# gsc74/DipGenie

Measured on AMD Instinct MI355X. Metric: dp_state_cells_per_s, higher is better.
Workload: dtype int32

## Files before the change

dipgenie_amd/csrc/dg_dp.hpp:

```cpp
#pragma once
#include <condition_variable>
#include <atomic>
#include <map>
#include <mutex>
#include <thread>
#include <tuple>

#include "dg_internal.hpp"

namespace dgi {

constexpr int32_t NEG_INF = INT32_MIN / 4;
constexpr uint32_t BP_NONE = 0xFFFFFFFFu;
constexpr int MAX_K = 1 << 15;
constexpr int BP_MAX_RANK = 255;
constexpr int COOP_MIN = 8;
constexpr int HEAVY_INLINE = 8;
constexpr int ROWX_MAX = 64;
constexpr int DELTA_PER_BLOCK = 256 * 16;
constexpr int DELTA_PAD = 8;
constexpr int32_t CHAIN_CORRUPT = INT32_MIN;
constexpr int64_t DELTA_MAX = 65535, COLOUR_LIST_MAX = 16383;
inline bool colour_lists_fit_delta(int64_t max_hom, int64_t max_het) {
    return max_hom <= COLOUR_LIST_MAX && max_het <= COLOUR_LIST_MAX && 2 * max_hom + 4 * max_het <= DELTA_MAX;
}

struct LevelDesc {
    int32_t a0, k;
    int32_t b0, k2;
    uint32_t in_base;
    int32_t T;
    int64_t delta_off;
    int64_t bp_off;
    int32_t grp_first, ngroups;
    int32_t dead_first, ndead;
    int64_t slot_first;
    int32_t fast_ok, nblocks;
    int32_t heavy_first, n_heavy;
    int32_t bp_wide, bp_nt;
    int64_t rowx_off;
    int32_t rowx_stride;
    int16_t heavy_in[HEAVY_INLINE];
    int32_t dmax;
};

struct TraceOut { int32_t value, s_het, n_e, overflow, corrupt, path_score; };
struct ChainState { int32_t i, j, r, value; };
struct BudgetSlot { int32_t chain, budget, planes, pad_; };
constexpr int BUDGET_SYNC_STRIDE = 128;
constexpr int BUDGET_HELPER_BLOCKS = 80;
struct ColourCsr { const int64_t *hom_off, *het_off; const int32_t *hom_col, *het_col; };

struct SweepArgs {
    const LevelDesc *descs;
    const uint32_t *in_off, *in_edge, *grp_begin;
    const int32_t *in_dst, *dead_cols;
    const uint16_t *delta, *delta_zero;
    char *ring;
    size_t slot_bytes, pad_bytes;
    uint16_t *bp;
    unsigned long long *digest;
    int RP;
    int *progress;
    int flip;
};

struct FastArgs {
    const uint4 *rowrec;
    const uint2 *slots;
    const uint32_t *in_edge, *rowx;
    const int32_t *dead_cols;
    const uint16_t *delta, *delta_zero;
    char *ring;
    uint16_t *bp;
    unsigned long long *digest;
    int RP, pad_bytes;
    uint32_t buf_bytes;
    uint32_t slot_bytes;
    int *progress;
    int flip;
#ifdef DG_SWEEP_PROBE
    unsigned long long *probe;
#endif
};

inline std::atomic<int> &dp_states_on_device(int device) { static std::atomic<int> n[64]; return n[device & 63]; }

struct SweepVariant {
    int rc;
    bool general, coop;
    int index() const;
    std::string name() const;
    bool exists() const;
    static int count();
    static SweepVariant at(int index);
};
constexpr int PAIR_MAX_INDEG = 8;
constexpr int PAIR_MAX_WIDTH = 255;
constexpr int PAIR_MAX_T = 2047;
constexpr int PAIR_RCS[] = {1, 2, 4};
constexpr int N_PAIR_RCS = (int)(sizeof PAIR_RCS / sizeof PAIR_RCS[0]);
constexpr int PAIR_BIG_MAX_INDEG = 32;
constexpr int PAIR_BIG_INLINE = 8;
constexpr uint32_t PAIR_ROW_BIG = 15;
struct PairDesc {
    int32_t l, nblocks;
    int32_t k0, k1, k2;
    int32_t dmax;
    int64_t row_first;
    int64_t slot_first;
    int32_t n_big, dmax_light;
    int64_t big_first;
    uint8_t big_in[PAIR_BIG_INLINE];
};
struct PairHist {
    int64_t n[2 * N_PAIR_RCS] = {};
    void add(const PairHist &o, int64_t sign = 1) { for (int q = 0; q < 2 * N_PAIR_RCS; ++q) n[q] += sign * o.n[q]; }
};

struct SweepHist {
    std::vector<int64_t> n = std::vector<int64_t>((size_t)SweepVariant::count(), 0);
    void add(const SweepHist &o, int64_t sign = 1) { for (size_t q = 0; q < n.size(); ++q) n[q] += sign * o.n[q]; }
};

struct DpOptions {
    int64_t side_stream = -1;
    int64_t plane_limit = 1;
    int64_t want_digest = 0;
    int64_t use_fast = 1;
    int64_t adaptive_rc = 1;
    int64_t use_coop = 1;
    int64_t max_blocks = 1024;
    int64_t segment_cells = 0;
    int64_t host_threads = 16;
    int64_t test_poison_level = 0, test_poison_byte = 0xFF;
    int64_t test_force_rc = 0;
    int64_t host_tables = 0;
    int64_t bp_nt_min_cells = 262144;
    int64_t graph_batch = -1;
    int64_t warm_ahead = 128;
    int64_t sync_every = 0;
    int64_t l2_prefetch = 6;
    int64_t use_lean_chain = 1;
    int64_t delta_overlap = 1;
    int64_t pf_far = 128;
    int64_t use_rowx = 1;
    int64_t delta_cap_entries = (int64_t)4 << 30;
    int64_t rc_cap = 65536, rc_t0_ns = 3000, rc_tg_ps = 20000, rc_tw_ps = 50;
    int64_t chunk_units_cfg = (int64_t)4 << 30;
    int64_t score_slab_bytes = (int64_t)256 << 20;
    int64_t partner_slab_bytes = (int64_t)4 << 30;
    int64_t partner_wide = 0;
    int64_t pair_levels = 1;
    int64_t pair_min = 4096;
    int64_t pair_fanin = 1;
    int64_t pair_fanin_min = 4096;
    int64_t pair_fanin_max_big = 4, pair_fanin_max_indeg = PAIR_BIG_MAX_INDEG;
    int64_t pair_digest = 0;
    int64_t test_force_pair_rc = 0;
    int64_t joint_state_bytes = (int64_t)8 << 30;
    int64_t genotype_table_bytes = (int64_t)256 << 20;
    int64_t genotype_table_lanes = 0;
    int64_t genotype_table_tile_keys = 2048;
    int64_t genotype_table_scan_tiles = 1024;
    int64_t objective_lds_bytes = 131072;
};

struct DpState {
    explicit DpState(int dev) : device(dev) { ++dp_states_on_device(device); }
    ~DpState() { --dp_states_on_device(device); }
    const int device;
    DpOptions opt;
    bool side_stream_ok() const { return opt.side_stream < 0 ? dp_states_on_device(device).load() <= 1 : opt.side_stream != 0; }
    DpState(const DpState &) = delete;
    DpState &operator=(const DpState &) = delete;
    int32_t nV = 0, L = 0, R = 0, RP = 0, cap = 0;
    bool loaded = false;
    bool lean_chain = false;
    std::vector<hipEvent_t> delta_piece_ev;
    std::vector<int32_t> delta_piece_level;
    int delta_piece_next = 0;
    hipStream_t pf_stream = nullptr;
    hipEvent_t pf_ev = nullptr;
    int pf_seq = 0;
    bool pf_active = false;
    int pf_tested = 0;
    std::vector<int> seg_begin;
    std::vector<int64_t> ckpt_off;
    bool graph_failed = false;
    typedef std::tuple<int, int, const void *, int> GraphKey;
    struct Batch { hipGraphExec_t exec = nullptr; SweepHist hist; PairHist pair_hist; int64_t n_launch = 0; int flips = 0; };
    std::map<GraphKey, Batch> graphs;
    bool all_fast = false;
    size_t state_alloc_bytes = 0;
    std::vector<LevelDesc> descs;
    uint64_t cells = 0, relaxations = 0, edge_pairs = 0, colour_entries = 0;
    int64_t total_units = 0, max_level_units = 0;
    int64_t max_level_cells = 0, delta_entries = 0, n_delta_blocks = 0, pad_front = 0;
    std::vector<int64_t> level_units;
    std::vector<int32_t> dwin_t, level_win;
    int cur_win = -1;
    std::vector<int32_t> dtrans_host;
    std::vector<int64_t> dblk_first_host;
    int64_t delta_buf_entries = 0;
    std::vector<int32_t> level_dmax;
    int64_t n_grp = 0, n_dead = 0, n_heavy_rows = 0, n_slot_records = 0, n_rowx_words = 0, n_dtrans = 0, n_edges = 0;
    DevBuf d_descs, d_in_off, d_in_edge, d_in_dst, d_hom_off, d_het_off, d_hom_col, d_het_col, d_eflag, d_eself;
    std::vector<PairDesc> pairs;
    std::vector<int32_t> pair_at;
    DevBuf d_pairs, d_pair_at, d_prow, d_pslots, d_pbig, d_pbig_rows;
    PairHist pair_hist;
    DevBuf d_delta, d_bp, d_ring, d_digest, d_dblk_first, d_dtrans, d_grp, d_dead, d_heavy, d_rowrec, d_rowx, d_slots, d_ckpt, d_pfctl;
#ifdef DG_SWEEP_PROBE
    DevBuf d_probe;
#endif
    std::vector<uint64_t> digest_host;
    SweepHist launch_hist;
    dg_dp_timing timing;
    hipEvent_t ev[4] = {nullptr, nullptr, nullptr, nullptr};
    struct Pool {
        std::mutex mu;
        std::condition_variable cv;
        std::vector<void *> chunks;
        size_t chunk_units = (size_t)DpOptions().chunk_units_cfg;
        size_t target = 0;
        size_t cap_chunks = 0;
        bool running = false, failed = false, paused = false;
        std::thread th;
    } pool;
    std::vector<int> chunk_begin;
    int seg_chunks = 1;
    DevBuf d_sink, d_ch_path, d_ch_state, d_ch_sync, d_ch_trace, d_ch_edges, d_ch_tab;
    std::vector<int32_t> sink_host;
    std::vector<BudgetSlot> tab_host;
    int n_groups = 0;
    mutable int walk_seq = 0;
    DevBuf d_sc_paths, d_sc_out, d_sc_err;
    DevBuf d_pt_pairs, d_pt_bud, d_pt_val, d_pt_out, d_pt_err, d_pt_bp, d_pt_scores;
    DevBuf d_pt_state;
    int32_t pt_route = 0;
    int64_t pt_route_cells = 0;
    DevBuf d_mg_levels, d_mg_vertex;
    bool run_ok = false;
    DevBuf d_ans_paths, d_ans_cnt;
    DevBuf d_cm_class, d_cm_out;
    bool ob_dict = false;
    int64_t ob_ch = 0, ob_ct = 0;
    DevBuf d_ob_hom_rank, d_ob_het_rank, d_ob_paths, d_ob_out, d_ob_err, d_ob_bits;
    int64_t jt_stats[8] = {0, 0, 0, 0, 0, 0, 0, 0};
    int64_t ph_stats[6] = {0, 0, 0, 0, 0, 0};
    int64_t phb_stats[10] = {0, 0, 0, 0, 0, 0, 0, 0, 0, 0};
    int64_t rb_stats[7] = {0, 0, 0, 0, 0, 0, 0};
    int64_t rbb_stats[9] = {0, 0, 0, 0, 0, 0, 0, 0, 0};
    DevBuf d_pins;
    bool run_pinned = false;
    int64_t pin_stats[5] = {0, 0, 0, 0, 0};
};

inline ColourCsr colour_csr(const DpState &S) {
    return ColourCsr{S.d_hom_off.as<int64_t>(), S.d_het_off.as<int64_t>(), S.d_hom_col.as<int32_t>(), S.d_het_col.as<int32_t>()};
}

void pool_request(DpState &S, int device, size_t target);
void pool_trim(DpState &S, size_t keep);
inline void pool_clear(DpState &S) { pool_trim(S, 0); }
void *pool_wait(DpState &S, size_t c);
struct PoolPause {
    DpState &S;
    explicit PoolPause(DpState &s);
    ~PoolPause();
};
void graphs_clear(DpState &S);
double wall_s();

int dp_load(dg_ctx *c, const dg_dp_graph *g);
int dp_build_tables_device(dg_ctx *c, const dg_dp_graph *g, DpState &S, std::vector<int32_t> &dtrans, std::vector<int64_t> &dblk_first, int &max_k);
int dp_table_digest(dg_ctx *c, uint64_t *out, int n);
int dp_build_pairs(dg_ctx *c, const dg_dp_graph *g, DpState &S);

void delta_launch_edge_flags(const DpState &S, hipStream_t s);
const uint16_t *delta_launch_window(DpState &S, int w, hipStream_t s);
const uint16_t *delta_launch_overlapped(DpState &S, hipStream_t s);
void delta_overlap_free(DpState &S);

struct SweepLaunch {
    SweepArgs A;
    FastArgs F;
    bool small_state = true;
    int rc_sel = 0;
    bool digest = false;
    int rp_active = 0;
    SweepHist hist;
    PairHist pair_hist;
    bool pairs_ok = false;
    int flip = 0;
};
void sweep_prepare(const DpState &S, SweepLaunch &X);
void sweep_init_state(const DpState &S, hipStream_t s);
int sweep_launch_level(const DpState &S, SweepLaunch &X, int l, hipStream_t s);
int sweep_launch_pair(const DpState &S, SweepLaunch &X, int l, hipStream_t s);
std::string pair_variant_name(int q);
void sweep_warm_tables(const DpState &S, const SweepLaunch &X, int q0, int q1, hipStream_t s);
int sweep_prefetch_begin(DpState &S, const SweepLaunch &X, int lb, int le, bool delta_resident, hipStream_t s);
void sweep_prefetch_end(DpState &S, int le, hipStream_t s);
void sweep_prefetch_free(DpState &S);

void trace_launch_warm_rows(const DpState &S, int lb, int le, hipStream_t s);
void trace_launch_chains(const DpState &S, int n, int l_hi, int l_lo, const uint16_t *bp_biased, const int32_t *final_val, hipStream_t s);
void trace_launch_finish_chain(const DpState &S, const uint2 *path, int32_t *edges, const ChainState *st, TraceOut *out, hipStream_t s);
void trace_debug_report(const DpState &S, int n);

void budgets_launch_sink_copy(const DpState &S, const int32_t *sink_state, hipStream_t s);
int budgets_reserve(DpState &S, int n);
int budgets_prepare(DpState &S, const int32_t *budgets, int n, hipStream_t s);
void budgets_launch_finish(const DpState &S, int n, hipStream_t s);
int budgets_find_chain(const char *fn, const DpState *S, int32_t budget, int &chain);
void budgets_launch_expand(const DpState &S, int chain, int swap, int32_t *out, int32_t *cnt, hipStream_t s);
int dp_get_answer_paths(dg_ctx *c, int32_t budget, int32_t *paths);

int dp_score_paths(dg_ctx *c, const int32_t *paths, int64_t n_pairs, dg_dp_pair_score *out);
int score_pair_blocks(const DpState &S);
void score_launch_pairs(const DpState &S, const int32_t *pairs, int64_t n, int32_t *out, unsigned long long *err, hipStream_t s);

int dp_objective_paths(dg_ctx *c, const int32_t *paths, int64_t n_pairs, dg_dp_pair_objective *out);
int dp_answer_objectives(dg_ctx *c, const int32_t *budgets, int32_t n_budgets, dg_dp_pair_objective *out);
int64_t objective_lds_limit(const dg_ctx *c);

int dp_best_partners(dg_ctx *c, const int32_t *given, int64_t n, const int32_t *budgets, int32_t *partners, dg_dp_partner *out);

int dp_partner_marginals(dg_ctx *c, const int32_t *given, int64_t n, const int32_t *budgets, dg_dp_level_margin *levels, int32_t *vertex_values);
int dp_call_margins(dg_ctx *c, int32_t budget, const int32_t *vertex_class, dg_dp_call_margin *levels, int32_t *paths);

struct PinSet {
    std::vector<int32_t> off;
    const dg_dp_pin *d_pins = nullptr;
    int64_t n_mask = 0, n_pairs_split = 0, n_batches_plain = 0;
    bool has(int l) const { return off[(size_t)l + 1] > off[(size_t)l]; }
    bool any_in(int l0, int l1) const { return off[(size_t)l1] > off[(size_t)l0]; }
};
int pins_prepare(const char *fn, const DpState &S, const dg_dp_pin *pins, int64_t n, PinSet &P, DevBuf &buf);
void pins_launch_mask(const DpState &S, PinSet &P, int level, int32_t *state, hipStream_t s);
void pins_launch_joint_mask(PinSet &P, int level, int32_t *state, int k, int planes, hipStream_t s);

int dp_genotype_margins(dg_ctx *c, bool pinned, const dg_dp_pin *pins, int64_t n_pins, const int32_t *called, int64_t n, int32_t budget, const int32_t *vertex_class,
                        dg_dp_genotype_margin *levels, int32_t *vertex_values, int32_t *best_value);
int dp_genotype_table(dg_ctx *c, bool pinned, const dg_dp_pin *pins, int64_t n_pins, int32_t budget, const int32_t *vertex_class, const int32_t *called, int64_t n,
                      dg_dp_genotype_margin *levels, int64_t *level_off, dg_dp_genotype_entry **entries, int64_t *n_entries, int32_t *best_value);
int dp_genotype_margins_budgets(dg_ctx *c, const dg_dp_pin *pins, int64_t n_pins, const int32_t *called, const int32_t *budgets, int64_t n, const int32_t *vertex_class,
                                dg_dp_genotype_margin *levels, int32_t *best_values);
int dp_genotype_stats(dg_ctx *c, int64_t *out, int n);
int dp_phase_margins(dg_ctx *c, const int32_t *called, int32_t budget, const int32_t *vertex_class, dg_dp_phase_margin *records, int64_t *n_records, int32_t *best_value);
int dp_phase_stats(dg_ctx *c, int64_t *out, int n);
int dp_phase_margins_budgets(dg_ctx *c, const int32_t *called, const int32_t *budgets, int64_t n, const int32_t *vertex_class, dg_dp_phase_margin *records, int64_t *record_off,
                             int32_t *best_values);
int dp_phase_budget_stats(dg_ctx *c, int64_t *out, int n);
int dp_recombination_margins(dg_ctx *c, int32_t budget, const int32_t *called, int64_t n, dg_dp_recombination_margin *records, int32_t *called_out, int32_t *best_value);
int dp_recombination_stats(dg_ctx *c, int64_t *out, int n);
int dp_recombination_margins_budgets(dg_ctx *c, const int32_t *budgets, int64_t n, const int32_t *called, dg_dp_recombination_margin *records, int32_t *called_out,
                                     int32_t *best_values);
int dp_recombination_budget_stats(dg_ctx *c, int64_t *out, int n);

}
```

dipgenie_amd/csrc/dg_dp_pairs.hip:

```cpp
#include <sched.h>

#include <algorithm>
#include <cstdlib>
#include <memory>

#include "dg_dp.hpp"

namespace dgi {

static int cpu_share() {
    int64_t n = (int64_t)std::max(1u, std::thread::hardware_concurrency());
    cpu_set_t set;
    if (sched_getaffinity(0, sizeof set, &set) == 0) n = std::min<int64_t>(n, std::max(1, CPU_COUNT(&set)));
    if (FILE *f = fopen("/sys/fs/cgroup/cpu.max", "r")) {
        long long quota = 0, period = 0;
        if (fscanf(f, "%lld %lld", &quota, &period) == 2 && quota > 0 && period > 0) n = std::min<int64_t>(n, (quota + period - 1) / period);
        fclose(f);
    }
    return (int)std::max<int64_t>(n, 1);
}

template <class F>
static void parallel_blocks(int64_t n, int64_t block, int nt, F f) {
    std::atomic<int64_t> next{0};
    auto work = [&]() {
        for (;;) {
            const int64_t b = next.fetch_add(block);
            if (b >= n) return;
            f(b, std::min(n, b + block));
        }
    };
    std::vector<std::thread> th;
    for (int t = 1; t < nt && (int64_t)t * block < n; ++t) th.emplace_back(work);
    work();
    for (std::thread &t : th) t.join();
}

int dp_build_pairs(dg_ctx *c, const dg_dp_graph *g, DpState &S) {
    S.pairs.clear(); S.pair_at.clear();
    S.d_pairs.release(); S.d_pair_at.release(); S.d_prow.release(); S.d_pslots.release(); S.d_pbig.release(); S.d_pbig_rows.release();
    const int L = S.L, nV = S.nV;
    if (!S.opt.pair_levels || (int64_t)(L - 1) / 2 < std::max<int64_t>(S.opt.pair_min, 1) || (int)S.dwin_t.size() != 2 || S.RP > 0x1FFF) return DG_OK;
    const double t0 = wall_s();
    std::vector<uint32_t> in_off((size_t)nV + 1, 0), in_edge((size_t)g->out_off[nV]);
    DG_HIP(hipMemcpyAsync(in_off.data(), S.d_in_off.p, 4 * in_off.size(), hipMemcpyDeviceToHost, c->stream));
    if (!in_edge.empty()) DG_HIP(hipMemcpyAsync(in_edge.data(), S.d_in_edge.p, 4 * in_edge.size(), hipMemcpyDeviceToHost, c->stream));
    DG_HIP(hipStreamSynchronize(c->stream));
    const int nt = (int)std::max<int64_t>(1, std::min<int64_t>({(int64_t)16, S.opt.host_threads, (int64_t)cpu_share()}));
    auto indeg = [&](int v) { return (int)(in_off[v + 1] - in_off[v]); };
    auto level_ok = [&](int l) {
        const LevelDesc &d = S.descs[l];
        return d.fast_ok == 1 && d.ndead == 0 && d.k2 <= PAIR_MAX_WIDTH && d.T <= PAIR_MAX_T && !d.bp_wide;
    };
    struct LevelSum { int32_t cmin, cmax, cmax_light, n_big; };
    std::vector<uint16_t> comp((size_t)nV, 0);
    std::vector<LevelSum> sum((size_t)L, LevelSum{0, 0, 0, 0});
    parallel_blocks(std::max(L - 2, 0), 512, nt, [&](int64_t q0, int64_t q1) {
        for (int l = (int)q0 + 2; l < (int)q1 + 2; ++l) {
            if (!level_ok(l - 1) || !level_ok(l)) continue;
            const LevelDesc &d = S.descs[l];
            LevelSum s{1 << 30, 0, 0, 0};
            for (int v = d.b0; v < d.b0 + d.k2; ++v) {
                int n = 0;
                for (uint32_t e = in_off[v]; e < in_off[v + 1]; ++e) n += indeg(d.a0 + (int)(in_edge[e] & 0x7FFFu));
                comp[(size_t)v] = (uint16_t)n;
                s.cmin = std::min(s.cmin, n); s.cmax = std::max(s.cmax, n);
                if (n > PAIR_MAX_INDEG) ++s.n_big; else s.cmax_light = std::max(s.cmax_light, n);
            }
            sum[(size_t)l] = s;
        }
    });
    const int max_big = (int)std::min<int64_t>(S.opt.pair_fanin_max_big, PAIR_MAX_WIDTH), max_indeg = (int)std::min<int64_t>(S.opt.pair_fanin_max_indeg, PAIR_BIG_MAX_INDEG);
    auto choose = [&](bool fanin, std::vector<PairDesc> &pairs, std::vector<int32_t> &at) {
        int64_t n_fanin = 0;
        pairs.clear(); at.assign((size_t)L, -1);
        for (int l = 2; l < L; ++l) {
            const LevelSum &s = sum[(size_t)l];
            if (s.cmin < 1) continue;
            if (s.cmax > PAIR_MAX_INDEG && !(fanin && s.cmax <= max_indeg && s.n_big <= max_big)) continue;
            const LevelDesc &d = S.descs[l];
            PairDesc p{};
            p.l = l; p.k0 = S.descs[l - 1].k; p.k1 = d.k; p.k2 = d.k2; p.dmax = s.cmax; p.n_big = s.n_big; p.dmax_light = s.cmax_light;
            n_fanin += s.n_big > 0;
            at[(size_t)l] = (int32_t)pairs.size(); at[(size_t)l - 1] = -2;
            pairs.push_back(p);
            ++l;
        }
        return n_fanin;
    };
    std::vector<int32_t> at;
    std::vector<PairDesc> pairs;
    int64_t n_fanin = choose(false, pairs, at);
    if (S.opt.pair_fanin) {
        std::vector<int32_t> at_f;
        std::vector<PairDesc> pairs_f;
        const int64_t nf = choose(true, pairs_f, at_f);
        if (nf >= std::max<int64_t>(S.opt.pair_fanin_min, 1)) { pairs.swap(pairs_f); at.swap(at_f); n_fanin = nf; }
    }
    if ((int64_t)pairs.size() < std::max<int64_t>(S.opt.pair_min, 1)) return DG_OK;
    const int64_t NP = (int64_t)pairs.size();
    parallel_blocks(NP, 256, nt, [&](int64_t q0, int64_t q1) {
        for (int64_t q = q0; q < q1; ++q) {
            PairDesc &p = pairs[(size_t)q];
            const LevelDesc &d2 = S.descs[p.l];
            uint32_t used = 0;
            int32_t nb = 1;
            for (int v = d2.b0; v < d2.b0 + d2.k2; ++v) {
                const uint32_t n = comp[(size_t)v];
                if (used + n > 64) { ++nb; used = 0; }
                used += n;
            }
            p.nblocks = nb;
        }
    });
    int64_t n_rows = 0, n_blocks = 0, n_big = 0;
    for (PairDesc &p : pairs) {
        p.row_first = n_rows * PAIR_MAX_INDEG; p.slot_first = n_blocks * 64; p.big_first = n_big;
        n_rows += p.k2; n_blocks += p.nblocks; n_big += p.n_big;
    }
    const size_t prow_words = 2 * (size_t)PAIR_MAX_INDEG * (size_t)n_rows, pslot_words = 4 * 64 * (size_t)n_blocks, pbig_words = 2 * (size_t)PAIR_BIG_MAX_INDEG * (size_t)n_big;
    std::unique_ptr<uint32_t[]> prow(new uint32_t[prow_words + 1]), pslots(new uint32_t[pslot_words + 1]), pbig(new uint32_t[pbig_words + 1]);
    std::unique_ptr<int32_t[]> big_rows(new int32_t[(size_t)n_big + 1]);
    parallel_blocks(NP, 64, nt, [&](int64_t q0, int64_t q1) {
        for (int64_t q = q0; q < q1; ++q) {
            PairDesc &p = pairs[(size_t)q];
            const LevelDesc &d2 = S.descs[p.l], &d1 = S.descs[p.l - 1];
            uint32_t *const pr = prow.get() + 2 * p.row_first, *const pb = pbig.get() + 2 * (size_t)PAIR_BIG_MAX_INDEG * (size_t)p.big_first;
            uint32_t *blk = pslots.get() + 4 * p.slot_first;
            int32_t *const br = big_rows.get() + p.big_first;
            uint32_t used = 0, maxdv = 1, h = 0;
            auto close_block = [&]() {
                uint32_t steps = 0;
                while ((1u << steps) < maxdv) ++steps;
                for (uint32_t s = used; s < 64; ++s) { blk[4 * s] = 0xFFFFFFFFu; blk[4 * s + 1] = 0; blk[4 * s + 2] = 0; blk[4 * s + 3] = 0; }
                for (uint32_t s = 0; s < 64; ++s) blk[4 * s + 2] |= steps << 16;
                blk += 4 * 64; used = 0; maxdv = 1;
            };
            for (int c2 = 0; c2 < d2.k2; ++c2) {
                const int v = d2.b0 + c2;
                const uint32_t n = comp[(size_t)v];
                const bool big = n > (uint32_t)PAIR_MAX_INDEG;
                if (used + n > 64) close_block();
                uint32_t *const light = pr + 2 * (size_t)PAIR_MAX_INDEG * (size_t)c2;
                uint32_t *const rec = big ? pb + 2 * (size_t)PAIR_BIG_MAX_INDEG * h : light;
                const uint32_t cap = big ? PAIR_BIG_MAX_INDEG : PAIR_MAX_INDEG, ru1_shift = big ? 27 : 25;
                uint32_t t = 0;
                for (uint32_t e2 = in_off[v]; e2 < in_off[v + 1]; ++e2) {
                    const uint32_t m = in_edge[e2] & 0x7FFFu, w2 = in_edge[e2] >> 31, r2 = e2 - in_off[v];
                    const int mv = d2.a0 + (int)m;
                    for (uint32_t e1 = in_off[mv]; e1 < in_off[mv + 1]; ++e1, ++t) {
                        const uint32_t src = in_edge[e1] & 0x7FFFu, w1 = in_edge[e1] >> 31, r1 = e1 - in_off[mv];
                        const uint32_t i2 = e2 - d2.in_base, i1 = e1 - d1.in_base;
                        rec[2 * t] = src | (w1 << 15) | (m << 16) | (w2 << 24) | (n << 25);
                        rec[2 * t + 1] = i2 | (i1 << 11) | (r2 << 22) | (r1 << ru1_shift);
                        uint32_t *const sl = blk + 4 * (used + t);
                        sl[0] = src | (w1 << 15) | (m << 16) | (w2 << 24);
                        sl[1] = i2 | (i1 << 16);
                        sl[2] = r2 | (r1 << 8) | ((uint32_t)c2 << 20);
                        sl[3] = 0;
                    }
                }
                for (; t < cap; ++t) { rec[2 * t] = n << 25; rec[2 * t + 1] = 0; }
                if (big) {
                    for (t = 0; t < (uint32_t)PAIR_MAX_INDEG; ++t) { light[2 * t] = PAIR_ROW_BIG << 25; light[2 * t + 1] = 0; }
                    br[h] = c2;
                    if (h < (uint32_t)PAIR_BIG_INLINE) p.big_in[h] = (uint8_t)c2;
                    ++h;
                }
                used += n; maxdv = std::max(maxdv, n);
            }
            close_block();
        }
    });
    auto up = [&](DevBuf &b, const void *src, size_t bytes) -> int {
        if (int rc = b.ensure(bytes + 16)) return rc;
        if (bytes) DG_HIP(hipMemcpyAsync(b.p, src, bytes, hipMemcpyHostToDevice, c->stream));
        return DG_OK;
    };
    if (int rc = up(S.d_pairs, pairs.data(), sizeof(PairDesc) * pairs.size())) return rc;
    if (int rc = up(S.d_pair_at, at.data(), 4 * at.size())) return rc;
    if (int rc = up(S.d_prow, prow.get(), 4 * prow_words)) return rc;
    if (int rc = up(S.d_pslots, pslots.get(), 4 * pslot_words)) return rc;
    if (int rc = up(S.d_pbig, pbig.get(), 4 * pbig_words)) return rc;
    if (int rc = up(S.d_pbig_rows, big_rows.get(), 4 * (size_t)n_big)) return rc;
    DG_HIP(hipStreamSynchronize(c->stream));
    if (getenv("DG_DEBUG"))
        fprintf(stderr, "[dipgenie_hip] load: %zu level pairs (%.1f %% of the launches), %lld of them with big rows (%lld big rows), composed tables %.1f MB, built in %.3f s by %d threads\n",
                pairs.size(), 100.0 * (double)pairs.size() / std::max(1, L - 1), (long long)n_fanin, (long long)n_big, 4e-6 * (double)(prow_words + pslot_words + pbig_words), wall_s() - t0, nt);
    S.pairs.swap(pairs); S.pair_at.swap(at);
    return DG_OK;
}

}
```

dipgenie_amd/csrc/dg_dp_run.hip:

```cpp
#include <algorithm>
#include <cstdlib>
#include <cstring>
#include <ctime>

#include "dg_dp.hpp"

namespace dgi {

constexpr int DELTA_NO_PIECES = 1 << 30;

double wall_s() { struct timespec ts; clock_gettime(CLOCK_MONOTONIC, &ts); return ts.tv_sec + 1e-9 * ts.tv_nsec; }

void graphs_clear(DpState &S) {
    for (auto &kv : S.graphs) if (kv.second.exec) (void)hipGraphExecDestroy(kv.second.exec);
    S.graphs.clear();
}

void dp_state_free(DpState *s) {
    if (!s) return;
    graphs_clear(*s);
    sweep_prefetch_free(*s);
    delta_overlap_free(*s);
    { std::unique_lock<std::mutex> lk(s->pool.mu); s->pool.target = 0; }
    s->pool.cv.notify_all();
    if (s->pool.th.joinable()) s->pool.th.join();
    const double tf0 = wall_s();
    for (void *q : s->pool.chunks) (void)hipFree(q);
    if (getenv("DG_DEBUG")) fprintf(stderr, "[dipgenie_hip] destroy: %zu lattice chunks freed in %.3f s\n", s->pool.chunks.size(), wall_s() - tf0);
    for (auto &e : s->ev) if (e) (void)hipEventDestroy(e);
    delete s;
}

void pool_request(DpState &S, int device, size_t target) {
    std::unique_lock<std::mutex> lk(S.pool.mu);
    S.pool.target = std::max(target, S.pool.chunks.size());
    if (S.pool.running || S.pool.chunks.size() >= S.pool.target) return;
    if (S.pool.th.joinable()) { lk.unlock(); S.pool.th.join(); lk.lock(); }
    S.pool.running = true;
    S.pool.failed = false;
    DpState *Sp = &S;
    S.pool.th = std::thread([Sp, device]() {
        (void)hipSetDevice(device);
        for (;;) {
            size_t bytes;
            {
                std::unique_lock<std::mutex> lk2(Sp->pool.mu);
                Sp->pool.cv.wait(lk2, [&] { return !Sp->pool.paused || Sp->pool.chunks.size() >= Sp->pool.target; });
                if (Sp->pool.chunks.size() >= Sp->pool.target) { Sp->pool.running = false; Sp->pool.cv.notify_all(); return; }
                bytes = Sp->pool.chunk_units * 2;
            }
            void *q = nullptr;
            const hipError_t e = hipMalloc(&q, bytes);
            std::unique_lock<std::mutex> lk2(Sp->pool.mu);
            if (e != hipSuccess) { (void)hipGetLastError(); Sp->pool.failed = true; Sp->pool.running = false; Sp->pool.cv.notify_all(); return; }
            Sp->pool.chunks.push_back(q);
            Sp->pool.cv.notify_all();
            lk2.unlock();
            std::this_thread::sleep_for(std::chrono::milliseconds(1));
        }
    });
}
PoolPause::PoolPause(DpState &s) : S(s) { std::unique_lock<std::mutex> lk(S.pool.mu); S.pool.paused = true; }
PoolPause::~PoolPause() { { std::unique_lock<std::mutex> lk(S.pool.mu); S.pool.paused = false; } S.pool.cv.notify_all(); }
void pool_trim(DpState &S, size_t keep) {
    { std::unique_lock<std::mutex> lk(S.pool.mu); S.pool.target = std::min(std::min(S.pool.target, keep), S.pool.chunks.size()); }
    S.pool.cv.notify_all();
    if (S.pool.th.joinable()) S.pool.th.join();
    std::unique_lock<std::mutex> lk(S.pool.mu);
    while (S.pool.chunks.size() > keep) { (void)hipFree(S.pool.chunks.back()); S.pool.chunks.pop_back(); }
    S.pool.running = false;
}
void *pool_wait(DpState &S, size_t c) {
    std::unique_lock<std::mutex> lk(S.pool.mu);
    S.pool.cv.wait(lk, [&] { return S.pool.chunks.size() > c || S.pool.failed || !S.pool.running; });
    return S.pool.chunks.size() > c ? S.pool.chunks[c] : nullptr;
}

namespace {

struct Run {
    dg_ctx *c;
    DpState &S;
    hipStream_t s;
    SweepLaunch X;
    int64_t n_launch = 0;
    int next_warm = 0;
    double host_enqueue_s = 0;
    int n_chains = 1;
    std::vector<uint16_t *> pool_base;
    PinSet *P;

    Run(dg_ctx *c_, DpState &S_, PinSet *P_ = nullptr) : c(c_), S(S_), s(c_->stream), P(P_) { sweep_prepare(S, X); }
    int n_win() const { return (int)S.dwin_t.size() - 1; }
    int32_t *state_ptr(int level) const { return (int32_t *)(S.d_ring.as<char>() + (size_t)((level & 1) ^ X.flip) * S.state_alloc_bytes) + S.pad_front; }
    size_t level_cells(int level) const {
        const int64_t k = level == 0 ? 1 : S.descs[level].k2;
        return (size_t)(k * k * S.RP);
    }
    void load_window(int w) { X.A.delta = X.F.delta = delta_launch_window(S, w, s); }

    int issue_levels(int l0, int l1, int lb, int le) {
        for (int l = l0; l < l1; ++l) {
            if (S.level_win[l] >= 0 && S.level_win[l] != S.cur_win) load_window(S.level_win[l]);
            if (S.opt.warm_ahead > 0 && l >= next_warm && (l == lb || !(S.pf_active && S.opt.pf_far > 0))) {
                const int q0 = l == lb ? l : (int)std::min<int64_t>(l + S.opt.warm_ahead, le), q1 = (int)std::min<int64_t>(l + 2 * S.opt.warm_ahead, le);
                if (q1 > q0) sweep_warm_tables(S, X, q0, q1, s);
            }
            if (l >= next_warm) next_warm = l + (int)std::max<int64_t>(S.opt.warm_ahead, 1);
            const bool pair_here = X.pairs_ok && l + 1 < l1 && S.pair_at[l + 1] >= 0;
            if (pair_here && !(P && P->has(l))) {
                if (S.level_win[l + 1] >= 0 && S.level_win[l + 1] != S.cur_win) load_window(S.level_win[l + 1]);
                if (int rc = sweep_launch_pair(S, X, ++l, s)) return rc;
            } else {
                if (pair_here) ++P->n_pairs_split;
                if (int rc = sweep_launch_level(S, X, l, s)) return rc;
            }
            ++n_launch;
            if (P && P->has(l)) pins_launch_mask(S, *P, l, state_ptr(l), s);
            if (S.opt.sync_every > 0 && n_launch % S.opt.sync_every == 0) DG_HIP(hipStreamSynchronize(s));
        }
        return DG_OK;
    }

    int sweep_range(int lb, int le, uint16_t *bp_biased) {
        X.A.bp = bp_biased; X.F.bp = bp_biased;
        next_warm = lb;
        if (int rc = sweep_prefetch_begin(S, X, lb, le, n_win() == 1, s)) return rc;
        const int64_t gb = S.opt.graph_batch >= 0 ? S.opt.graph_batch : 1000;
        for (int l0 = lb; l0 < le;) {
            const int pf_key = ((S.pf_active && S.opt.pf_far > 0) ? 1 : 0) | (X.flip << 1) | (X.rp_active << 2);
            const bool graph_ok = gb > 0 && n_win() == 1 && S.opt.sync_every == 0 && !S.graph_failed;
            const int l1 = graph_ok ? (int)std::min<int64_t>((int64_t)l0 + gb, le) : le;
            const bool pinned_batch = P && P->any_in(l0, l1);
            if (graph_ok && pinned_batch) ++P->n_batches_plain;
            const bool use_graph = graph_ok && !pinned_batch;
            while (S.delta_piece_next < (int)S.delta_piece_level.size() && S.delta_piece_level[S.delta_piece_next] < l1) {
                DG_HIP(hipStreamWaitEvent(s, S.delta_piece_ev[S.delta_piece_next], 0));
                ++S.delta_piece_next;
            }
            const DpState::GraphKey key(l0, l1, (const void *)bp_biased, pf_key);
            DpState::Batch *slot = nullptr;
            bool capturing = false;
            if (use_graph) {
                slot = &S.graphs[key];
                if (slot->exec) {
                    DG_HIP(hipGraphLaunch(slot->exec, s));
                    X.hist.add(slot->hist); X.pair_hist.add(slot->pair_hist);
                    n_launch += slot->n_launch; X.flip ^= slot->flips; l0 = l1;
                    continue;
                }
                if (hipStreamBeginCapture(s, hipStreamCaptureModeThreadLocal) == hipSuccess) capturing = true;
                else { (void)hipGetLastError(); S.graph_failed = true; continue; }
            }
            const int64_t n_launch_before = n_launch;
            const SweepHist hist_before = X.hist;
            const PairHist pair_hist_before = X.pair_hist;
            const int flip_before = X.flip;
            if (int rc = issue_levels(l0, l1, lb, le)) {
                if (capturing) {
                    hipGraph_t cg = nullptr;
                    (void)hipStreamEndCapture(s, &cg);
                    if (cg) (void)hipGraphDestroy(cg);
                    (void)hipGetLastError();
                    S.graphs.erase(key);
                }
                return rc;
            }
            if (capturing) {
                hipGraph_t cg = nullptr;
                const bool ok = hipStreamEndCapture(s, &cg) == hipSuccess && cg && hipGraphInstantiate(&slot->exec, cg, nullptr, nullptr, 0) == hipSuccess;
                if (cg) (void)hipGraphDestroy(cg);
                if (!ok) {
                    (void)hipGetLastError();
                    slot->exec = nullptr; S.graph_failed = true; n_launch = n_launch_before; X.hist = hist_before; X.pair_hist = pair_hist_before; X.flip = flip_before;
                    continue;
                }
                slot->hist = X.hist;
                slot->hist.add(hist_before, -1);
                slot->pair_hist = X.pair_hist;
                slot->pair_hist.add(pair_hist_before, -1);
                slot->n_launch = n_launch - n_launch_before; slot->flips = X.flip ^ flip_before;
                DG_HIP(hipGraphLaunch(slot->exec, s));
            }
            l0 = l1;
        }
        sweep_prefetch_end(S, le, s);
        return DG_OK;
    }

    int wait_for_chunks() {
        if (S.d_bp.p) return DG_OK;
        const double tw0 = wall_s();
        const size_t need = (size_t)std::min(S.seg_chunks, (int)S.chunk_begin.size() - 1);
        if (!pool_wait(S, need - 1)) { set_error("back-pointer lattice: hipMalloc of a %.1f GB chunk failed", S.pool.chunk_units * 2 / 1e9); return DG_ERR_OOM; }
        std::unique_lock<std::mutex> lk(S.pool.mu);
        for (size_t q = 0; q < need; ++q) pool_base.push_back((uint16_t *)S.pool.chunks[q]);
        if (getenv("DG_DEBUG")) fprintf(stderr, "[dipgenie_hip] run: waited %.3f s for lattice chunks\n", wall_s() - tw0);
        return DG_OK;
    }

    std::tuple<int, int, uint16_t *> chunk(int ch, int c0) const {
        const int lb = S.d_bp.p ? 1 : S.chunk_begin[ch], le = S.d_bp.p ? S.L : S.chunk_begin[ch + 1];
        return {lb, le, (S.d_bp.p ? S.d_bp.as<uint16_t>() : pool_base[ch - c0]) - S.descs[lb].bp_off};
    }

    int sweep_and_walk(int c0, int c1, bool from_sink, bool mark_forward_end) {
        for (int ch = c0; ch < c1; ++ch) {
            const auto [lb, le, bp] = chunk(ch, c0);
            const double th0 = wall_s();
            if (int rc = sweep_range(lb, le, bp)) return rc;
            host_enqueue_s += wall_s() - th0;
        }
        if (mark_forward_end) { DG_HIP(hipEventRecord(S.ev[2], s)); budgets_launch_sink_copy(S, state_ptr(S.L - 1), s); }
        if (S.opt.test_poison_level > 0 && S.opt.test_poison_level < S.L)
            for (int ch = c0; ch < c1; ++ch) {
                const auto [lb, le, bp] = chunk(ch, c0);
                const int lp = (int)S.opt.test_poison_level;
                if (lp >= lb && lp < le) DG_HIP(hipMemsetAsync(bp + S.descs[lp].bp_off, (int)S.opt.test_poison_byte, 2 * (size_t)S.level_units[lp], s));
            }
        for (int ch = c1 - 1; ch >= c0; --ch) {
            const auto [lb, le, bp] = chunk(ch, c0);
            trace_launch_warm_rows(S, lb, le, s);
            const int32_t *final_val = from_sink && ch == c1 - 1 ? state_ptr(S.L - 1) : (const int32_t *)nullptr;
            trace_launch_chains(S, n_chains, le - 1, lb, bp, final_val, s);
        }
        return DG_OK;
    }

    int forward_and_trace() {
        const int n_seg = (int)S.seg_begin.size() - 1, n_chunks_all = (int)S.chunk_begin.size() - 1;
        DG_HIP(hipEventRecord(S.ev[0], s));
        S.cur_win = -1;
        S.delta_piece_next = DELTA_NO_PIECES;
        if (n_win() == 1 && S.n_delta_blocks > 0) X.A.delta = X.F.delta = delta_launch_overlapped(S, s);
        DG_HIP(hipEventRecord(S.ev[1], s));
        if (S.opt.want_digest) DG_HIP(hipMemsetAsync(S.d_digest.p, 0, 8 * (size_t)S.L, s));
#ifdef DG_SWEEP_PROBE
        {
            std::vector<unsigned long long> init((size_t)S.L * 8, 0ULL);
            for (int l = 0; l < S.L; ++l) init[(size_t)l * 8] = ~0ULL;
            DG_HIP(hipMemcpy(S.d_probe.p, init.data(), 8 * init.size(), hipMemcpyHostToDevice));
        }
#endif
        sweep_init_state(S, s);
        X.pairs_ok = !S.pairs.empty() && S.opt.pair_levels && n_seg == 1 && n_win() == 1 && (!X.digest || S.opt.pair_digest) && S.opt.use_fast && S.opt.adaptive_rc && S.opt.test_force_rc == 0 &&
                     X.small_state && X.rp_active == S.RP;
        if (n_seg == 1) {
            if (int rc = sweep_and_walk(0, S.d_bp.p ? 1 : n_chunks_all, true, true)) return rc;
        } else {
            int64_t planes_swept = 0;
            for (int sg = 0; sg < n_seg; ++sg) {
                if (sg > 0)
                    DG_HIP(hipMemcpyAsync(S.d_ckpt.as<int32_t>() + S.ckpt_off[sg], state_ptr(S.seg_begin[sg] - 1),
                                          4 * level_cells(S.seg_begin[sg] - 1), hipMemcpyDeviceToDevice, s));
                if (int rc = sweep_range(S.seg_begin[sg], S.seg_begin[sg + 1], nullptr)) return rc;
            }
            DG_HIP(hipEventRecord(S.ev[2], s));
            budgets_launch_sink_copy(S, state_ptr(S.L - 1), s);
            X.digest = false;
            for (int sg = n_seg - 1; sg >= 0; --sg) {
                const int lb = S.seg_begin[sg];
                if (sg > 0)
                    DG_HIP(hipMemcpyAsync(state_ptr(lb - 1), S.d_ckpt.as<int32_t>() + S.ckpt_off[sg], 4 * level_cells(lb - 1), hipMemcpyDeviceToDevice, s));
                else
                    sweep_init_state(S, s);
                const int c0 = sg * S.seg_chunks, c1 = std::min(n_chunks_all, c0 + S.seg_chunks);
                if (int rc = sweep_and_walk(c0, c1, sg == n_seg - 1, false)) return rc;
                if (S.opt.plane_limit && sg > 0) {
                    std::vector<ChainState> cs((size_t)n_chains);
                    DG_HIP(hipMemcpyAsync(cs.data(), S.d_ch_state.p, sizeof(ChainState) * cs.size(), hipMemcpyDeviceToHost, s));
                    DG_HIP(hipStreamSynchronize(s));
                    int planes = 1;
                    for (const ChainState &q : cs) {
                        if (q.value == NEG_INF) continue;
                        planes = std::max(planes, (q.value != CHAIN_CORRUPT && q.r >= 0 && q.r < S.RP) ? q.r + 1 : S.RP);
                    }
                    X.rp_active = planes;
                    planes_swept += (int64_t)planes * (S.seg_begin[sg] - S.seg_begin[sg - 1]);
                }
            }
            if (getenv("DG_DEBUG") && S.opt.plane_limit) fprintf(stderr, "[dipgenie_hip] run: second pass swept %.1f %% of the (level, plane) pairs before the last segment\n",
                                                              100.0 * (double)planes_swept / std::max(1.0, (double)S.RP * (S.seg_begin[n_seg - 1] - 1)));
        }
        budgets_launch_finish(S, n_chains, s);
        DG_HIP(hipEventRecord(S.ev[3], s));
        DG_HIP(hipGetLastError());
        return DG_OK;
    }
};

}

static int emit_result(const DpState &S, const TraceOut &to, const int32_t *edges, dg_dp_result *res, int budget) {
    char who[32] = "";
    if (budget >= 0) snprintf(who, sizeof who, " (budget %d)", budget);
    if (to.value == CHAIN_CORRUPT || to.corrupt) { set_error("back-pointer lattice is corrupt: the chain walk left its level (a level was not swept?)%s", who); return DG_ERR_STATE; }
    if (to.value != NEG_INF && to.path_score != to.value) {
        set_error("traceback path scores %d but the DP value is %d: sweep, lattice and walk disagree%s", to.path_score, to.value, who); return DG_ERR_STATE;
    }
    if (to.overflow || to.n_e > S.cap) { set_error("traceback edge list overflow (%d > %d)%s", to.n_e, S.cap, who); return DG_ERR_STATE; }
    res->value = to.value; res->s_het = to.s_het;
    res->cells = S.cells; res->relaxations = S.relaxations;
    std::vector<int> order(to.n_e);
    for (int q = 0; q < to.n_e; ++q) order[q] = q;
    std::stable_sort(order.begin(), order.end(), [&](int a, int b) { return edges[a] < edges[b]; });
    int n1 = 0, n2 = 0;
    for (int q : order) {
        const int from = edges[S.cap + q], tov = edges[2 * S.cap + q];
        if (edges[3 * S.cap + q] == 0) { if (n1 < res->cap && res->p1_from && res->p1_to) { res->p1_from[n1] = from; res->p1_to[n1] = tov; } ++n1; }
        else { if (n2 < res->cap && res->p2_from && res->p2_to) { res->p2_from[n2] = from; res->p2_to[n2] = tov; } ++n2; }
    }
    res->n_p1 = n1; res->n_p2 = n2;
    return DG_OK;
}

static int dp_run(dg_ctx *c, const int32_t *budgets, int n_budgets, dg_dp_result *res, bool name_budget, PinSet *P = nullptr) {
    DpState &S = *c->dp;
    Run run(c, S, P);
    hipStream_t s = c->stream;
    if (int rc = run.wait_for_chunks()) return rc;
    std::vector<TraceOut> to((size_t)n_budgets);
    std::vector<int32_t> edges(4 * (size_t)S.cap * (size_t)n_budgets);
    S.run_ok = false;
    S.run_pinned = P != nullptr;
    if (int rc = budgets_prepare(S, budgets, n_budgets, s)) return rc;
    run.n_chains = n_budgets;
    S.sink_host.clear();
    const int rc_run = run.forward_and_trace();
    S.launch_hist = run.X.hist;
    S.pair_hist = run.X.pair_hist;
    if (rc_run) return rc_run;
    DG_HIP(hipMemcpyAsync(to.data(), S.d_ch_trace.p, sizeof(TraceOut) * to.size(), hipMemcpyDeviceToHost, s));
    DG_HIP(hipMemcpyAsync(edges.data(), S.d_ch_edges.p, 4 * edges.size(), hipMemcpyDeviceToHost, s));
    std::vector<int32_t> sink((size_t)S.RP);
    DG_HIP(hipMemcpyAsync(sink.data(), S.d_sink.p, 4 * sink.size(), hipMemcpyDeviceToHost, s));
    if (S.opt.want_digest) {
        S.digest_host.assign(S.L, 0);
        DG_HIP(hipMemcpyAsync(S.digest_host.data(), S.d_digest.p, 8 * (size_t)S.L, hipMemcpyDeviceToHost, s));
    }
    DG_HIP(hipStreamSynchronize(s));
    S.sink_host.swap(sink);
#ifdef DG_SWEEP_PROBE
    if (const char *po = getenv("DG_PROBE_OUT")) {
        std::vector<unsigned long long> pr((size_t)S.L * 8);
        DG_HIP(hipMemcpy(pr.data(), S.d_probe.p, 8 * pr.size(), hipMemcpyDeviceToHost));
        if (FILE *f = fopen(po, "wb")) { fwrite(pr.data(), 8, pr.size(), f); fclose(f); }
    }
#endif
    if (getenv("DG_DEBUG") && S.lean_chain) trace_debug_report(S, n_budgets);
    if (getenv("DG_DEBUG") && S.pf_stream) {
        int w[4] = {0, 0, 0, 0};
        if (hipStreamSynchronize(S.pf_stream) == hipSuccess && hipMemcpy(w, S.d_pfctl.p, sizeof w, hipMemcpyDeviceToHost) == hipSuccess)
            fprintf(stderr, "[dipgenie_hip] run: L2 table prefetcher covered %d levels (since load)\n", w[2]);
    }
    if (getenv("DG_DEBUG"))
        fprintf(stderr, "[dipgenie_hip] run: host issued %lld sweep launches in %.1f ms (%.2f us each)\n", (long long)run.n_launch, 1e3 * run.host_enqueue_s,
                1e6 * run.host_enqueue_s / (double)std::max<int64_t>(run.n_launch, 1));
    DG_HIP(hipEventElapsedTime(&S.timing.delta_ms, S.ev[0], S.ev[1]));
    DG_HIP(hipEventElapsedTime(&S.timing.forward_ms, S.ev[1], S.ev[2]));
    DG_HIP(hipEventElapsedTime(&S.timing.traceback_ms, S.ev[2], S.ev[3]));
    DG_HIP(hipEventElapsedTime(&S.timing.total_ms, S.ev[0], S.ev[3]));
    S.timing.n_forward_launches = run.n_launch;
    S.timing.n_segments = (int32_t)S.seg_begin.size() - 1;
    S.timing.n_chunks = (int32_t)S.chunk_begin.size() - 1;
    for (int q = 0; q < n_budgets; ++q)
        if (int rc = emit_result(S, to[q], edges.data() + 4 * (size_t)S.cap * (size_t)q, res + q, name_budget ? budgets[q] : -1)) return rc;
    S.run_ok = true;
    return DG_OK;
}

static int check_budgets(const char *fn, const DpState *Sp, const int32_t *budgets, int32_t n, const dg_dp_result *results) {
    if (!Sp || !Sp->loaded) { set_error("%s: no graph loaded", fn); return DG_ERR_STATE; }
    if (!budgets || !results || n <= 0) { set_error("%s: budgets, results and n_budgets > 0 are required", fn); return DG_ERR_ARG; }
    std::vector<char> seen((size_t)Sp->RP, 0);
    for (int q = 0; q < n; ++q) {
        const int b = budgets[q];
        if (b < 0 || b > Sp->R) { set_error("%s: budget %d (entry %d) outside 0..%d, the R of the loaded graph", fn, b, q, Sp->R); return DG_ERR_ARG; }
        if (seen[b]) { set_error("%s: budget %d listed twice", fn, b); return DG_ERR_ARG; }
        seen[b] = 1;
        if (results[q].cap < b + 2) { set_error("%s: results[%d].cap = %d, budget %d needs %d", fn, q, results[q].cap, b, b + 2); return DG_ERR_ARG; }
    }
    return DG_OK;
}

static int dp_run_budgets(dg_ctx *c, const int32_t *budgets, int32_t n, dg_dp_result *results) {
    if (int rc = check_budgets("dg_dp_run_budgets", c->dp, budgets, n, results)) return rc;
    return dp_run(c, budgets, n, results, true);
}

static int dp_run_pinned(dg_ctx *c, const dg_dp_pin *pins, int64_t n_pins, const int32_t *budgets, int32_t n, dg_dp_result *results) {
    if (n_pins == 0) return dp_run_budgets(c, budgets, n, results);
    if (int rc = check_budgets("dg_dp_run_pinned", c->dp, budgets, n, results)) return rc;
    DpState &S = *c->dp;
    if (S.opt.want_digest) {
        set_error("dg_dp_run_pinned: option digest is 1: the sweep accumulates a level's digest before the level's mask runs, so the digest would describe another DP");
        return DG_ERR_STATE;
    }
    PinSet P;
    if (int rc = pins_prepare("dg_dp_run_pinned", S, pins, n_pins, P, S.d_pins)) return rc;
    const int rc = dp_run(c, budgets, n, results, true, &P);
    int64_t n_levels = 0;
    for (int l = 1; l < S.L; ++l) n_levels += P.has(l);
    const int64_t st[5] = {n_pins, n_levels, P.n_mask, P.n_pairs_split, P.n_batches_plain};
    memcpy(S.pin_stats, st, sizeof st);
    return rc;
}

static int dp_run_single(dg_ctx *c, dg_dp_result *res) {
    if (!c->dp || !c->dp->loaded) { set_error("dg_dp_run: no graph loaded"); return DG_ERR_STATE; }
    if (!res) { set_error("dg_dp_run: null result"); return DG_ERR_ARG; }
    const int32_t budget = c->dp->R;
    return dp_run(c, &budget, 1, res, false);
}

}

extern "C" int dg_dp_load_graph(dg_ctx *c, const dg_dp_graph *g) {
    if (int rc = dgi::bind(c)) return rc;
    return dgi::dp_load(c, g);
}
extern "C" int dg_dp_run(dg_ctx *c, dg_dp_result *r) {
    if (int rc = dgi::bind(c)) return rc;
    return dgi::dp_run_single(c, r);
}
extern "C" int dg_dp_run_budgets(dg_ctx *c, const int32_t *budgets, int32_t n_budgets, dg_dp_result *results) {
    if (int rc = dgi::bind(c)) return rc;
    return dgi::dp_run_budgets(c, budgets, n_budgets, results);
}
extern "C" int dg_dp_run_pinned(dg_ctx *c, const dg_dp_pin *pins, int64_t n_pins, const int32_t *budgets, int32_t n_budgets, dg_dp_result *results) {
    if (int rc = dgi::bind(c)) return rc;
    return dgi::dp_run_pinned(c, pins, n_pins, budgets, n_budgets, results);
}
extern "C" int dg_dp_get_pin_stats(dg_ctx *c, int64_t *out, int n) {
    if (!c || !c->dp) { dgi::set_error("dg_dp_get_pin_stats: no state"); return DG_ERR_STATE; }
    if (!out || n < 5) { dgi::set_error("dg_dp_get_pin_stats: out with n >= 5 entries is required"); return DG_ERR_ARG; }
    memcpy(out, c->dp->pin_stats, sizeof c->dp->pin_stats);
    return DG_OK;
}
extern "C" int dg_dp_get_budget_values(dg_ctx *c, int32_t *out, int32_t n) {
    if (!c || !c->dp || !out) { dgi::set_error("dg_dp_get_budget_values: no state"); return DG_ERR_STATE; }
    const std::vector<int32_t> &v = c->dp->sink_host;
    if (v.empty()) { dgi::set_error("dg_dp_get_budget_values: no completed dg_dp_run / dg_dp_run_budgets on the loaded graph"); return DG_ERR_STATE; }
    if (n < (int32_t)v.size()) { dgi::set_error("dg_dp_get_budget_values: out has %d entries, R + 1 = %zu needed", n, v.size()); return DG_ERR_ARG; }
    memcpy(out, v.data(), 4 * v.size());
    return DG_OK;
}
extern "C" int dg_dp_solve_diploid(dg_ctx *c, const dg_dp_graph *g, dg_dp_result *r) {
    if (int rc = dg_dp_load_graph(c, g)) return rc;
    return dg_dp_run(c, r);
}
extern "C" int dg_dp_prealloc(dg_ctx *c, int64_t bytes) {
    if (int rc = dgi::bind(c)) return rc;
    if (!c->dp) c->dp = new dgi::DpState(c->device);
    dgi::DpState &S = *c->dp;
    if (S.pool.chunk_units != (size_t)S.opt.chunk_units_cfg) { dgi::pool_clear(S); S.pool.chunk_units = (size_t)S.opt.chunk_units_cfg; }
    const size_t chunk_bytes = S.pool.chunk_units * 2;
    if (S.pool.cap_chunks == 0) {
        size_t free_b = 0, total_b = 0;
        DG_HIP(hipMemGetInfo(&free_b, &total_b));
        S.pool.cap_chunks = std::max<size_t>(1, (size_t)(0.6 * (double)free_b) / chunk_bytes);
    }
    const size_t want_chunks = bytes > 0 ? std::min(((size_t)bytes + chunk_bytes - 1) / chunk_bytes, S.pool.cap_chunks) : S.pool.cap_chunks;
    dgi::pool_request(S, c->device, want_chunks);
    return DG_OK;
}
extern "C" int dg_dp_get_timing(dg_ctx *c, dg_dp_timing *t) {
    if (!c || !c->dp || !t) { dgi::set_error("dg_dp_get_timing: no state"); return DG_ERR_STATE; }
    *t = c->dp->timing;
    return DG_OK;
}
extern "C" int dg_dp_get_level_digest(dg_ctx *c, uint64_t *out, int64_t n) {
    if (!c || !c->dp || !out) { dgi::set_error("dg_dp_get_level_digest: no state"); return DG_ERR_STATE; }
    if ((int64_t)c->dp->digest_host.size() != n) { dgi::set_error("digest not collected (set option digest=1) or size mismatch"); return DG_ERR_STATE; }
    memcpy(out, c->dp->digest_host.data(), 8 * (size_t)n);
    return DG_OK;
}
extern "C" int dg_dp_get_table_digest(dg_ctx *c, uint64_t *out, int n) {
    if (int rc = dgi::bind(c)) return rc;
    return dgi::dp_table_digest(c, out, n);
}
extern "C" int dg_dp_get_launch_profile(dg_ctx *c, char *buf, int cap) {
    if (!c || !c->dp || !buf || cap < 2) { dgi::set_error("dg_dp_get_launch_profile: no state"); return DG_ERR_STATE; }
    std::string out;
    for (int q = 0; q < dgi::SweepVariant::count(); ++q)
        if (const int64_t n = c->dp->launch_hist.n[(size_t)q]) out += (out.empty() ? "" : " ") + dgi::SweepVariant::at(q).name() + ':' + std::to_string(n);
    if ((int)out.size() + 1 > cap) { dgi::set_error("dg_dp_get_launch_profile: buffer too small (%zu needed)", out.size() + 1); return DG_ERR_ARG; }
    memcpy(buf, out.c_str(), out.size() + 1);
    return DG_OK;
}
extern "C" int dg_dp_get_pair_profile(dg_ctx *c, char *buf, int cap) {
    if (!c || !c->dp || !buf || cap < 2) { dgi::set_error("dg_dp_get_pair_profile: no state"); return DG_ERR_STATE; }
    std::string out;
    for (int q = 0; q < 2 * dgi::N_PAIR_RCS; ++q)
        if (const int64_t n = c->dp->pair_hist.n[q]) out += (out.empty() ? "" : " ") + dgi::pair_variant_name(q) + ':' + std::to_string(n);
    if ((int)out.size() + 1 > cap) { dgi::set_error("dg_dp_get_pair_profile: buffer too small (%zu needed)", out.size() + 1); return DG_ERR_ARG; }
    memcpy(buf, out.c_str(), out.size() + 1);
    return DG_OK;
}
extern "C" int dg_dp_list_pair_variants(char *buf, int cap) {
    std::string out;
    for (int q = 0; q < dgi::N_PAIR_RCS; ++q) out += (out.empty() ? "" : " ") + dgi::pair_variant_name(q);
    if (!buf || (int)out.size() + 1 > cap) { dgi::set_error("dg_dp_list_pair_variants: buffer too small (%zu needed)", out.size() + 1); return DG_ERR_ARG; }
    memcpy(buf, out.c_str(), out.size() + 1);
    return DG_OK;
}
extern "C" int dg_dp_list_sweep_variants(char *buf, int cap) {
    std::string out;
    for (int q = 0; q < dgi::SweepVariant::count(); ++q)
        if (dgi::SweepVariant::at(q).exists()) out += (out.empty() ? "" : " ") + dgi::SweepVariant::at(q).name();
    if (!buf || (int)out.size() + 1 > cap) { dgi::set_error("dg_dp_list_sweep_variants: buffer too small (%zu needed)", out.size() + 1); return DG_ERR_ARG; }
    memcpy(buf, out.c_str(), out.size() + 1);
    return DG_OK;
}
typedef dgi::DpOptions DpO;
static const struct DpOptionKey { const char *key; int64_t DpO::*field; int64_t lo; bool nonpos_is_default; } dp_option_keys[] = {
    {"digest", &DpO::want_digest, 0, false}, {"fast", &DpO::use_fast, 0, false}, {"adaptive_rc", &DpO::adaptive_rc, 0, false}, {"coop", &DpO::use_coop, 0, false},
    {"sync_every", &DpO::sync_every, 0, false}, {"rc_t0_ns", &DpO::rc_t0_ns, 0, false}, {"rc_tg_ps", &DpO::rc_tg_ps, 0, false}, {"rc_tw_ps", &DpO::rc_tw_ps, 0, false},
    {"rc_cap", &DpO::rc_cap, 0, true}, {"max_blocks", &DpO::max_blocks, 0, true}, {"bp_nt_min_cells", &DpO::bp_nt_min_cells, 0, false}, {"warm_ahead", &DpO::warm_ahead, 0, false},
    {"graph_batch", &DpO::graph_batch, -1, false}, {"l2_prefetch", &DpO::l2_prefetch, 0, false}, {"delta_overlap", &DpO::delta_overlap, 0, false}, {"pf_far", &DpO::pf_far, 0, false},
    {"side_stream", &DpO::side_stream, -1, false}, {"plane_limit", &DpO::plane_limit, 0, false}, {"test_poison_level", &DpO::test_poison_level, 0, false},
    {"test_poison_byte", &DpO::test_poison_byte, 0, false}, {"test_force_rc", &DpO::test_force_rc, 0, false}, {"pair_digest", &DpO::pair_digest, 0, false}, {"test_force_pair_rc", &DpO::test_force_pair_rc, 0, false},
    {"score_slab_bytes", &DpO::score_slab_bytes, 0, true}, {"partner_slab_bytes", &DpO::partner_slab_bytes, 0, true},
    {"partner_wide", &DpO::partner_wide, 0, false},
    {"joint_state_bytes", &DpO::joint_state_bytes, 0, true},
    {"genotype_table_bytes", &DpO::genotype_table_bytes, 0, true}, {"genotype_table_lanes", &DpO::genotype_table_lanes, 0, false},
    {"genotype_table_tile_keys", &DpO::genotype_table_tile_keys, 256, true}, {"genotype_table_scan_tiles", &DpO::genotype_table_scan_tiles, 64, true},
    {"objective_lds_bytes", &DpO::objective_lds_bytes, 0, true},
    {"rowx", &DpO::use_rowx, 0, false}, {"lean_chain", &DpO::use_lean_chain, 0, false}, {"segment_cells", &DpO::segment_cells, 0, false},
    {"host_threads", &DpO::host_threads, 1, false}, {"host_tables", &DpO::host_tables, 0, false}, {"delta_cap_entries", &DpO::delta_cap_entries, 0, true},
    {"pair_levels", &DpO::pair_levels, 0, false}, {"pair_min", &DpO::pair_min, 1, false}, {"pair_fanin", &DpO::pair_fanin, 0, false}, {"pair_fanin_min", &DpO::pair_fanin_min, 1, false},
    {"pair_fanin_max_big", &DpO::pair_fanin_max_big, 0, false}, {"pair_fanin_max_indeg", &DpO::pair_fanin_max_indeg, 0, false},
    {"lattice_chunk_cells", &DpO::chunk_units_cfg, 1, false},
};
static int dp_option(dg_ctx *c, const char *what, const char *key, const int64_t *set, int64_t *get) {
    if (!c || !key || (!set && !get)) { dgi::set_error("%s: null", what); return DG_ERR_ARG; }
    if (!c->dp) c->dp = new dgi::DpState(c->device);
    dgi::DpState &S = *c->dp;
    if (set) dgi::graphs_clear(S);
    for (const DpOptionKey &o : dp_option_keys) {
        if (strcmp(key, o.key)) continue;
        if (!set) { *get = S.opt.*o.field; return DG_OK; }
        int64_t v = *set;
        if (o.field == &DpO::chunk_units_cfg) {
            if (v < o.lo) { dgi::set_error("lattice_chunk_cells must be positive"); return DG_ERR_ARG; }
            dgi::pool_clear(S);
            v = (int64_t)(S.pool.chunk_units = ((size_t)v + 1) & ~(size_t)1);
        }
        if (o.field == &DpO::objective_lds_bytes) v = std::min(v, dgi::objective_lds_limit(c));
        if (o.field == &DpO::partner_wide) v = std::min<int64_t>(v, 2);
        if (o.field == &DpO::genotype_table_tile_keys && v > 0) v = std::min<int64_t>(std::max<int64_t>(v / 256, 1) * 256, 2048);
        if (o.field == &DpO::genotype_table_scan_tiles && v > 0) v = std::min<int64_t>(std::max<int64_t>(v / 64, 1) * 64, 1024);
        S.opt.*o.field = o.nonpos_is_default && v <= 0 ? DpO().*o.field : v < o.lo ? o.lo : v;
        return DG_OK;
    }
    dgi::set_error("unknown option %s", key);
    return DG_ERR_ARG;
}
extern "C" int dg_dp_set_option(dg_ctx *c, const char *key, int64_t v) { return dp_option(c, "dg_dp_set_option", key, &v, nullptr); }
extern "C" int dg_dp_get_option(dg_ctx *c, const char *key, int64_t *value) { return dp_option(c, "dg_dp_get_option", key, nullptr, value); }
```

dipgenie_amd/csrc/dg_dp_sweep.hip:

```cpp
#include <algorithm>
#include <cmath>
#include <type_traits>

#include "dg_dp.hpp"

namespace dgi {

#define DG_SLOT(LEVEL) ((LEVEL) & 1)

constexpr unsigned long long DIGEST_PRED_MUL = 0x9E3779B97F4A7C15ULL;

__device__ __forceinline__ void store_bp_nt(uint16_t *p, uint32_t v) { asm volatile("global_store_short %0, %1, off nt" ::"v"(p), "v"(v) : "memory"); }
__device__ __forceinline__ uint32_t ord_rank(int eu, int ev) { return ((uint32_t)(BP_MAX_RANK - eu) << 8) | (uint32_t)(BP_MAX_RANK - ev); }

__device__ __forceinline__ unsigned long long digest_term(int value, unsigned long long o, uint32_t pred_i, uint32_t pred_j) {
    return (unsigned long long)(uint32_t)(value + 1) * (o + 1) +
           DIGEST_PRED_MUL * ((((unsigned long long)pred_i << 15) | pred_j) + 1ULL) * (o + 1);
}

__device__ __forceinline__ int lane_down1(int x) { return __builtin_amdgcn_update_dpp(x, x, 0x130 , 0xF, 0xF, false); }
__device__ __forceinline__ int lane_up1(int x) { return __builtin_amdgcn_update_dpp(x, x, 0x138 , 0xF, 0xF, false); }

struct LevelHead {
    const uint4 *rowrec_l;
    const uint2 *slots_l;
    const uint32_t *rowx_l;
    const int32_t *cur;
    const uint16_t *dm;
    int rowx_stride, RP, k, pad_bytes, dT;
    uint32_t buf_bytes;
};

__device__ __forceinline__ __amdgpu_buffer_rsrc_t state_rsrc(const int32_t *padded_base, uint32_t bytes) {
    return __builtin_amdgcn_make_buffer_rsrc((void *)padded_base, 0, bytes, 0x00020000);
}

__device__ __forceinline__ void publish_level(int *progress, int lvl) {
    if ((blockIdx.x | blockIdx.y | blockIdx.z) == 0 && threadIdx.x == 0) __hip_atomic_store(progress, lvl, __ATOMIC_RELAXED, __HIP_MEMORY_SCOPE_AGENT);
}

__device__ __forceinline__ uint32_t ord_word(int i, int j, int wu, int wv) {
    return ((uint32_t)(0x7FFF - i) << 17) | ((uint32_t)(0x7FFF - j) << 2) | ((uint32_t)wu << 1) | (uint32_t)wv;
}
__device__ __forceinline__ uint32_t bp_from_ord(uint32_t o) {
    const uint32_t i = 0x7FFFu - (o >> 17), j = 0x7FFFu - ((o >> 2) & 0x7FFFu);
    return i | (j << 15) | (((o >> 1) & 1u) << 30) | ((o & 1u) << 31);
}
template <int RC, bool DIGEST>
__device__ __forceinline__ void sweep_level_pairs(const SweepArgs &A, int lvl, int wave_id, int n_waves) {
    const LevelDesc d = A.descs[lvl];
    const int RP = A.RP;
    const int32_t *__restrict__ cur = (const int32_t *)(A.ring + (size_t)(DG_SLOT(lvl - 1) ^ A.flip) * A.slot_bytes + A.pad_bytes);
    int32_t *__restrict__ nxt = (int32_t *)(A.ring + (size_t)(DG_SLOT(lvl) ^ A.flip) * A.slot_bytes + A.pad_bytes);
    const int lane = threadIdx.x & 63;
    const int nchunk = (RP + RC - 1) / RC;
    const int64_t ntask = (int64_t)d.k2 * d.ngroups * nchunk;
    const bool has_delta = d.delta_off >= 0;
    const uint16_t *dm = has_delta ? A.delta + d.delta_off : A.delta_zero;
    const int dT = has_delta ? d.T : 0, dmask = has_delta ? -1 : 0;
    const uint32_t *gb = A.grp_begin + d.grp_first;
    unsigned long long dsum = 0;
    for (int64_t task = wave_id; task < ntask; task += n_waves) {
        const int g = (int)(task % d.ngroups);
        const int64_t rest = task / d.ngroups;
        const int rc = (int)(rest % nchunk), i2 = (int)(rest / nchunk);
        const int r0 = rc * RC;
        const uint32_t gbeg = gb[g], gend = gb[g + 1];
        const uint32_t eu0 = A.in_off[d.b0 + i2], eu1 = A.in_off[d.b0 + i2 + 1];
        int bval[RC];
        uint32_t bord[RC];
#pragma unroll
        for (int q = 0; q < RC; ++q) { bval[q] = NEG_INF; bord[q] = 0; }
        int j2 = -1 - lane;
        for (uint32_t cb = gbeg; cb < gend; cb += 64) {
            const uint32_t ev = cb + lane;
            const bool act = ev < gend;
            int j = 0, wv = 0, evr = 0;
            if (act) {
                const uint32_t pv = A.in_edge[ev];
                j = (int)(pv & 0x7FFFFFFFu); wv = (int)(pv >> 31);
                const int cv = A.in_dst[ev];
                j2 = cv - d.b0;
                if (!d.bp_wide) evr = (int)(ev - A.in_off[cv]);
            }
            const int dcol = (int)(ev - d.in_base) & dmask;
            for (uint32_t eu = eu0; eu < eu1; ++eu) {
                const uint32_t pu = A.in_edge[eu];
                const int i = (int)(pu & 0x7FFFFFFFu), wu = (int)(pu >> 31);
                if (act) {
                    const int w = wu + wv;
                    const int dl = (int)dm[(int64_t)(eu - d.in_base) * dT + dcol];
                    const uint32_t ord = d.bp_wide ? ord_word(i, j, wu, wv) : ord_rank((int)(eu - eu0), evr);
                    const int32_t *base = cur + ((int64_t)i * RP + (r0 - w)) * d.k + j;
                    int vals[RC];
#pragma unroll
                    for (int q = 0; q < RC; ++q) vals[q] = base[q * d.k];
#pragma unroll
                    for (int q = 0; q < RC; ++q) {
                        const int cand = vals[q] + dl;
                        const bool ok = (r0 + q < RP) & (r0 + q - w >= 0) & (vals[q] != NEG_INF);
                        const bool take = ok & ((cand > bval[q]) | ((cand == bval[q]) & (ord > bord[q])));
                        bval[q] = take ? cand : bval[q];
                        bord[q] = take ? ord : bord[q];
                    }
                }
            }
        }
        const int span = (int)min(gend - gbeg, 64u);
        for (int s = 1; s < span; s <<= 1) {
            const int oj2 = __shfl_down(j2, s);
            const bool same = (lane + s < 64) & (oj2 == j2);
#pragma unroll
            for (int q = 0; q < RC; ++q) {
                const int ov = __shfl_down(bval[q], s);
                const uint32_t oo = (uint32_t)__shfl_down((int)bord[q], s);
                const bool take = same & ((ov > bval[q]) | ((ov == bval[q]) & (oo > bord[q])));
                bval[q] = take ? ov : bval[q];
                bord[q] = take ? oo : bord[q];
            }
        }
        const int pj2 = __shfl_up(j2, 1);
        const bool head = (j2 >= 0) & ((lane == 0) | (pj2 != j2));
        if (head) {
#pragma unroll
            for (int q = 0; q < RC; ++q) {
                const int r2 = r0 + q;
                if (r2 < RP) {
                    const int64_t idx = ((int64_t)i2 * RP + r2) * d.k2 + j2;
                    nxt[idx] = bval[q];
                    if (A.bp) {
                        if (d.bp_wide) __builtin_nontemporal_store((uint32_t)(bval[q] == NEG_INF ? BP_NONE : bp_from_ord(bord[q])), (uint32_t *)(A.bp + d.bp_off + 2 * idx));
                        else __builtin_nontemporal_store((uint16_t)~bord[q], &A.bp[d.bp_off + idx]);
                    }
                    if (DIGEST && bval[q] != NEG_INF) {
                        const unsigned long long o = ((unsigned long long)r2 * d.k2 + i2) * d.k2 + j2;
                        uint32_t pi, pj;
                        if (d.bp_wide) { const uint32_t h = bp_from_ord(bord[q]); pi = h & 0x7FFFu; pj = (h >> 15) & 0x7FFFu; }
                        else {
                            const uint32_t ru = BP_MAX_RANK - (bord[q] >> 8), rv = BP_MAX_RANK - (bord[q] & 0xFFu);
                            pi = A.in_edge[eu0 + ru] & 0x7FFFFFFFu;
                            pj = A.in_edge[A.in_off[d.b0 + j2] + rv] & 0x7FFFFFFFu;
                        }
                        dsum += digest_term(bval[q], o, pi, pj);
                    }
                }
            }
        }
        if (g == 0 && d.ndead > 0) {
            for (int t = lane; t < d.ndead * RC; t += 64) {
                const int q = t % RC, c = A.dead_cols[d.dead_first + t / RC];
                if (r0 + q < RP) {
                    const int64_t idx = ((int64_t)i2 * RP + r0 + q) * d.k2 + c;
                    nxt[idx] = NEG_INF;
                    if (A.bp) {
                        if (d.bp_wide) __builtin_nontemporal_store((uint32_t)(BP_NONE), (uint32_t *)(A.bp + d.bp_off + 2 * idx));
                        else __builtin_nontemporal_store((uint16_t)0xFFFFu, &A.bp[d.bp_off + idx]);
                    }
                }
            }
        }
    }
    if (DIGEST && dsum) atomicAdd(&A.digest[lvl], dsum);
}

template <int RC, bool DIGEST>
__global__ __launch_bounds__(256) void dp_sweep_kernel(SweepArgs A, int lvl) {
    sweep_level_pairs<RC, DIGEST>(A, lvl, (int)(blockIdx.x * 4 + (threadIdx.x >> 6)), (int)(gridDim.x * 4));
}

__global__ void dp_init_kernel(int32_t *cur, int RP) {
    const int r = (int)(blockIdx.x * blockDim.x + threadIdx.x);
    if (r < RP) cur[r] = 0;
}


template <int RC>
__device__ __forceinline__ void relax_select(const int (&vals)[RC], int dl, uint32_t ord, int r0, int w, int RP,
                                             int (&bval)[RC], uint32_t (&bord)[RC]) {
#pragma unroll
    for (int q = 0; q < RC; ++q) {
        const int cand = vals[q] + dl;
        const bool ok = (r0 + q < RP) & (r0 + q - w >= 0) & (vals[q] != NEG_INF);
        const bool take = ok & ((cand > bval[q]) | ((cand == bval[q]) & (ord > bord[q])));
        bval[q] = take ? cand : bval[q];
        bord[q] = take ? ord : bord[q];
    }
}

__device__ __forceinline__ void merge_best(int ov, uint32_t oo, bool same, int &bv, uint32_t &bo) {
    const bool take = same & ((ov > bv) | ((ov == bv) & (oo > bo)));
    bv = take ? ov : bv;
    bo = take ? oo : bo;
}

#ifdef DG_SWEEP_PROBE
#define DG_PROBE_BEGIN unsigned long long pq[6] = {0, 0, 0, 0, 0, 0}; \
    const bool probe_on = A.probe != nullptr && blockIdx.x == 0 && blockIdx.y == 0 && (threadIdx.x >> 6) == 0 && (int)blockIdx.z < d.k2;
#define DG_PROBE(q) do { if (probe_on) { asm volatile("s_waitcnt vmcnt(0) lgkmcnt(0)" ::: "memory"); pq[q] = __builtin_amdgcn_s_memrealtime(); } } while (0)
#define DG_PROBE_END do { if (probe_on && (threadIdx.x & 63) == 0) { \
        atomicMin(&A.probe[(size_t)lvl * 8 + 0], pq[0]); atomicMax(&A.probe[(size_t)lvl * 8 + 1], pq[5]); \
        if ((int)blockIdx.z == d.k2 / 2) for (int q = 0; q < 6; ++q) A.probe[(size_t)lvl * 8 + 2 + q] = pq[q]; } } while (0)
#else
#define DG_PROBE_BEGIN
#define DG_PROBE(q) do { } while (0)
#define DG_PROBE_END do { } while (0)
#endif

template <int RC, bool DIGEST, bool GENERAL, int COOP>
__device__ __forceinline__ void sweep_task(const LevelHead &H, const FastArgs &A, const LevelDesc &d, __amdgpu_buffer_rsrc_t cur_rsrc,
                                           int32_t *__restrict__ nxt, int i2, int g, int r0, int lvl, int part = 0, uint2 *ex = nullptr) {
    const int lane = threadIdx.x & 63;
    const int RP = H.RP;
    DG_PROBE_BEGIN
    DG_PROBE(0);
    const uint4 rr = H.rowrec_l[i2];
    uint2 sl = H.slots_l[g * 64 + lane];
    const bool rowx = !GENERAL && H.rowx_stride > 0;
    uint32_t mypu = 0;
    if (rowx && lane < H.rowx_stride) mypu = H.rowx_l[i2 * H.rowx_stride + lane];
    int steps = __builtin_amdgcn_readfirstlane((int)(sl.y >> 28));
    const int j2 = (sl.x != 0xFFFFFFFFu) ? (int)((sl.x >> 16) & 0x7FFFu) : -1 - lane;
    int nblk = 1;
    if (GENERAL) {
        if (steps == 14) return;
        if (steps == 15) {
            const int col = __builtin_amdgcn_readfirstlane(j2);
            nblk = ((int)H.rowrec_l[col].y + 63) >> 6;
            steps = 6;
        }
    }
    const uint16_t *dm = H.dm;
    const int dT = H.dT;
    const bool has_delta = dT != 0;
    const int du = (int)rr.y;
    if (COOP == 1 && du > COOP_MIN) return;
    DG_PROBE(1);
    const int t_lo = COOP == 2 ? (du * part) >> 2 : 0, t_hi = COOP == 2 ? (du * (part + 1)) >> 2 : du;
    int bval[RC];
    uint32_t bord[RC];
#pragma unroll
    for (int q = 0; q < RC; ++q) { bval[q] = NEG_INF; bord[q] = 0; }
    const int64_t erow0 = (int64_t)rr.x * dT;
    const int rowbytes = H.k * 4;
    bool act = false;
    for (int blk = 0; blk < (GENERAL ? nblk : 1); ++blk) {
        if (GENERAL && blk > 0) sl = H.slots_l[(g + blk) * 64 + lane];
        const bool actb = sl.x != 0xFFFFFFFFu;
        act |= actb;
        const int j = (int)(sl.x & 0x7FFFu), wv = (int)((sl.x >> 15) & 1u);
        const int dcol = has_delta ? (int)(sl.y & 0x000FFFFFu) : 0;
        const int evr = (int)((sl.y >> 20) & 0xFFu);
        if (du <= 2) {
            if (actb && du > 0) {
                const int ia = (int)(rr.z & 0x7FFFu), wa = (int)(rr.z >> 31) + wv;
                const int ib = (int)(rr.w & 0x7FFFu), wb = (int)(rr.w >> 31) + wv;
                const int offa = ((ia * RP + (r0 - wa)) * H.k + j) * 4 + H.pad_bytes;
                const int offb = ((ib * RP + (r0 - wb)) * H.k + j) * 4 + H.pad_bytes;
                int va[RC], vb[RC];
                const int dla = (int)dm[erow0 + dcol];
                int dlb = 0;
#pragma unroll
                for (int q = 0; q < RC; ++q)
                    va[q] = __builtin_amdgcn_raw_buffer_load_b32(cur_rsrc, offa + q * rowbytes, 0, 0);
                if (du == 2) {
                    dlb = (int)dm[erow0 + dT + dcol];
#pragma unroll
                    for (int q = 0; q < RC; ++q)
                        vb[q] = __builtin_amdgcn_raw_buffer_load_b32(cur_rsrc, offb + q * rowbytes, 0, 0);
                }
                relax_select<RC>(va, dla, ord_rank(0, evr), r0, wa, RP, bval, bord);
                if (du == 2) relax_select<RC>(vb, dlb, ord_rank(1, evr), r0, wb, RP, bval, bord);
            }
        } else {
            constexpr int U = GENERAL ? (RC >= 4 ? 2 : 4) : (RC >= 8 ? 2 : (RC >= 4 ? 4 : 8));
            for (int c0 = GENERAL ? t_lo : 0; c0 < t_hi; c0 += GENERAL ? 64 : (1 << 30)) {
                const int tb = GENERAL ? c0 : t_lo, te = GENERAL ? min(c0 + 64, t_hi) : t_hi;
                if (!rowx) { mypu = 0; if (c0 + lane < te) mypu = A.in_edge[rr.x + c0 + lane]; }
                for (int t = tb; t < te; t += U) {
                    uint32_t wmask = 0;
                    if (actb) {
                        int vals[U][RC], dl[U];
#pragma unroll
                        for (int u = 0; u < U; ++u) {
                            if (t + u < te) {
                                const uint32_t p = (uint32_t)__builtin_amdgcn_readlane((int)mypu, t + u - c0);
                                wmask |= (p >> 31) << u;
                                const int iu = (int)(p & 0x7FFFFFFFu), w = (int)(p >> 31) + wv;
                                const int off = ((iu * RP + (r0 - w)) * H.k + j) * 4 + H.pad_bytes;
                                dl[u] = (int)dm[erow0 + (int64_t)(t + u) * dT + dcol];
#pragma unroll
                                for (int q = 0; q < RC; ++q)
                                    vals[u][q] = __builtin_amdgcn_raw_buffer_load_b32(cur_rsrc, off + q * rowbytes, 0, 0);
                            }
                        }
#pragma unroll
                        for (int u = 0; u < U; ++u) {
                            if (t + u < te) {
                                const int wu = (int)((wmask >> u) & 1u);
                                relax_select<RC>(vals[u], dl[u], ord_rank(t + u, evr), r0, wu + wv, RP, bval, bord);
                            }
                        }
                    }
                }
            }
        }
    }
    DG_PROBE(2);
    if (COOP == 2) {
        if (part > 0) {
#pragma unroll
            for (int q = 0; q < RC; ++q) ex[((part - 1) * RC + q) * 64 + lane] = make_uint2((uint32_t)bval[q], bord[q]);
        }
        __syncthreads();
        if (part > 0) return;
#pragma unroll
        for (int p = 0; p < 3; ++p) {
#pragma unroll
            for (int q = 0; q < RC; ++q) {
                const uint2 o = ex[(p * RC + q) * 64 + lane];
                merge_best((int)o.x, o.y, true, bval[q], bord[q]);
            }
        }
    }
    if (steps > 0) {
        const int oj2 = lane_down1(j2);
        const bool same = (lane + 1 < 64) & (oj2 == j2);
#pragma unroll
        for (int q = 0; q < RC; ++q) merge_best(lane_down1(bval[q]), (uint32_t)lane_down1((int)bord[q]), same, bval[q], bord[q]);
    }
    for (int st = 1, sh = 2; st < steps; ++st, sh <<= 1) {
        const int oj2 = __shfl_down(j2, sh);
        const bool same = (lane + sh < 64) & (oj2 == j2);
#pragma unroll
        for (int q = 0; q < RC; ++q) merge_best(__shfl_down(bval[q], sh), (uint32_t)__shfl_down((int)bord[q], sh), same, bval[q], bord[q]);
    }
    const int pj2 = lane_up1(j2);
    const bool head = act & ((lane == 0) | (pj2 != j2));
    unsigned long long dsum = 0;
    DG_PROBE(3);
    if (head) {
#pragma unroll
        for (int q = 0; q < RC; ++q) {
            const int r2 = r0 + q;
            if (r2 < RP) {
                const int idx = (i2 * RP + r2) * d.k2 + j2;
                nxt[idx] = bval[q];
                if (A.bp) { if (d.bp_nt) store_bp_nt(&A.bp[d.bp_off + idx], ~bord[q]); else A.bp[d.bp_off + idx] = (uint16_t)~bord[q]; }
                if (DIGEST && bval[q] != NEG_INF) {
                    const unsigned long long o = ((unsigned long long)r2 * d.k2 + i2) * d.k2 + j2;
                    const uint32_t ru = BP_MAX_RANK - (bord[q] >> 8), rv = BP_MAX_RANK - (bord[q] & 0xFFu);
                    const uint32_t pi = A.in_edge[rr.x + ru] & 0x7FFFFFFFu;
                    const uint32_t pj = A.in_edge[H.rowrec_l[j2].x + rv] & 0x7FFFFFFFu;
                    dsum += digest_term(bval[q], o, pi, pj);
                }
            }
        }
    }
    if (g == 0 && d.ndead > 0) {
        for (int t = lane; t < d.ndead * RC; t += 64) {
            const int q = t % RC, c = A.dead_cols[d.dead_first + t / RC];
            if (r0 + q < RP) {
                const int64_t idx = ((int64_t)i2 * RP + r0 + q) * d.k2 + c;
                nxt[idx] = NEG_INF;
                if (A.bp) { if (d.bp_nt) store_bp_nt(&A.bp[d.bp_off + idx], 0xFFFFu); else A.bp[d.bp_off + idx] = (uint16_t)0xFFFFu; }
            }
        }
    }
    if (DIGEST && dsum) atomicAdd(&A.digest[lvl], dsum);
#ifdef DG_SWEEP_PROBE
    if (probe_on) pq[4] = __builtin_amdgcn_s_memrealtime();
    DG_PROBE(5);
    DG_PROBE_END;
#endif
}

#ifndef DG_PLAIN_WG
#define DG_PLAIN_WG 256
#endif
#define DG_PLAIN_GW ((DG_PLAIN_WG / 64) < 4 ? (DG_PLAIN_WG / 64) : 4)
#define DG_PLAIN_CH ((DG_PLAIN_WG / 64) / DG_PLAIN_GW)
template <int RC, bool DIGEST, bool GENERAL>
__global__ __launch_bounds__(DG_PLAIN_WG) void dp_sweep_fast_kernel(const uint4 *rowrec_l, const uint2 *slots_l, const uint32_t *rowx_l, const int32_t *cur, const uint16_t *dm,
                                                            int rowx_stride, int nblocks, int rp_k, int pad_bytes, int dT, uint32_t buf_bytes,
                                                            FastArgs A, LevelDesc d, int lvl) {
    const LevelHead H{rowrec_l, slots_l, rowx_l, cur, dm, rowx_stride, rp_k & 0x1FFF, rp_k >> 13, pad_bytes, dT, buf_bytes};
    publish_level(A.progress, lvl);
    const int wv = (int)(threadIdx.x >> 6);
    const int g = (int)blockIdx.x * DG_PLAIN_GW + (wv % DG_PLAIN_GW);
    const int r0 = ((int)blockIdx.y * DG_PLAIN_CH + wv / DG_PLAIN_GW) * RC;
    if (g >= nblocks || r0 >= (rp_k & 0x1FFF)) return;
    int32_t *nxt = (int32_t *)(A.ring + (size_t)(DG_SLOT(lvl) ^ A.flip) * A.slot_bytes + A.pad_bytes);
    sweep_task<RC, DIGEST, GENERAL, 0>(H, A, d, state_rsrc(cur, buf_bytes), nxt, (int)blockIdx.z, g, r0, lvl);
}

template <int RC, bool DIGEST, bool GENERAL>
__global__ __launch_bounds__(256) void dp_sweep_coop_kernel(const uint4 *rowrec_l, const uint2 *slots_l, const uint32_t *rowx_l, const int32_t *cur,
                                                            int rowx_stride, int nblocks, int n_heavy, int rp_k, unsigned long long heavy_lo,
                                                            unsigned long long heavy_hi,
                                                            FastArgs A, LevelDesc d, int lvl, const uint16_t *dm, int dT, const int32_t *__restrict__ heavy_rows) {
    const LevelHead H{rowrec_l, slots_l, rowx_l, cur, dm, rowx_stride, rp_k & 0x1FFF, rp_k >> 13, A.pad_bytes, dT, A.buf_bytes};
    publish_level(A.progress, lvl);
    int32_t *nxt = (int32_t *)(A.ring + (size_t)(DG_SLOT(lvl) ^ A.flip) * A.slot_bytes + A.pad_bytes);
    const int r0 = (int)blockIdx.y * RC;
    const int zc = 4 * n_heavy;
    if ((int)blockIdx.z < zc) {
        __shared__ uint2 ex[3 * RC * 64];
        const int hz = (int)blockIdx.z;
        const int g = (int)blockIdx.x * 4 + (hz & 3);
        if (g >= nblocks) return;
        const int h = hz >> 2;
        int i2;
        if (h < 4) i2 = (int)((heavy_lo >> (16 * h)) & 0xFFFFu);
        else if (h < HEAVY_INLINE) i2 = (int)((heavy_hi >> (16 * (h - 4))) & 0xFFFFu);
        else i2 = heavy_rows[d.heavy_first + h];
        sweep_task<RC, DIGEST, GENERAL, 2>(H, A, d, state_rsrc(cur, A.buf_bytes), nxt, i2, g, r0, lvl, (int)(threadIdx.x >> 6), ex);
        return;
    }
    const int g = (int)blockIdx.x * 4 + (int)(threadIdx.x >> 6);
    if (g >= nblocks) return;
    sweep_task<RC, DIGEST, GENERAL, 1>(H, A, d, state_rsrc(cur, A.buf_bytes), nxt, (int)blockIdx.z - zc, g, r0, lvl);
}

template <int RC>
__device__ __forceinline__ void relax_pair(const int (&vals)[RC], int dl, uint32_t ord, uint32_t mid, int r0, int w, int RP,
                                           int (&bval)[RC], uint32_t (&bord)[RC], uint32_t (&bmid)[RC]) {
#pragma unroll
    for (int q = 0; q < RC; ++q) {
        const int cand = vals[q] + dl;
        const bool ok = (r0 + q < RP) & (r0 + q - w >= 0) & (vals[q] != NEG_INF);
        const bool take = ok & ((cand > bval[q]) | ((cand == bval[q]) & (ord > bord[q])));
        bval[q] = take ? cand : bval[q];
        bord[q] = take ? ord : bord[q];
        bmid[q] = take ? mid : bmid[q];
    }
}
__device__ __forceinline__ void merge_best_pair(int ov, uint32_t oo, uint32_t om, bool same, int &bv, uint32_t &bo, uint32_t &bm) {
    const bool take = same & ((ov > bv) | ((ov == bv) & (oo > bo)));
    bv = take ? ov : bv;
    bo = take ? oo : bo;
    bm = take ? om : bm;
}

struct PairHead {
    const uint4 *pslots_l;
    const int32_t *cur;
    const uint16_t *dm1, *dm2;
    int RP, k0, pad_bytes, dT1, dT2;
    uint32_t buf_bytes;
};

template <int RC, bool DIGEST, int COOP>
__device__ __forceinline__ void pair_task(const PairHead &H, const uint2 *recs, int32_t *__restrict__ nxt, uint16_t *__restrict__ bp1, uint16_t *__restrict__ bp2, int kk, int nt,
                                          int i2, int g, int r0, int lvl, unsigned long long *digest, int part = 0, uint4 *ex = nullptr) {
    const int lane = threadIdx.x & 63;
    const int RP = H.RP, k0 = H.k0, pad_bytes = H.pad_bytes, dT1 = H.dT1, dT2 = H.dT2;
    const uint16_t *dm1 = H.dm1, *dm2 = H.dm2;
    constexpr int NREC = COOP == 2 ? PAIR_BIG_MAX_INDEG : PAIR_MAX_INDEG, RU1_SHIFT = COOP == 2 ? 27 : 25, RANK_MASK = COOP == 2 ? 31 : 7;
    const uint2 rec = recs[lane & (NREC - 1)];
    const uint4 sl = H.pslots_l[g * 64 + lane];
    const __amdgpu_buffer_rsrc_t cur_rsrc = state_rsrc(H.cur, H.buf_bytes);
    const int du = __builtin_amdgcn_readfirstlane((int)(rec.x >> 25)) & (COOP == 2 ? 0x3F : 0xF);
    if (COOP == 1 && du > PAIR_MAX_INDEG) return;
    const int t_lo = COOP == 2 ? (du * part) >> 2 : 0, t_hi = COOP == 2 ? (du * (part + 1)) >> 2 : du;
    const int steps = __builtin_amdgcn_readfirstlane((int)(sl.z >> 16)) & 0xF;
    const bool act = sl.x != 0xFFFFFFFFu;
    const int j = (int)(sl.x & 0x7FFFu), wv = (int)((sl.x >> 15) & 1u) + (int)((sl.x >> 24) & 1u);
    const uint32_t lanemid = (((sl.x >> 16) & 0xFFu) << 8) | ((sl.x >> 24) & 1u);
    const int j2 = act ? (int)((sl.z >> 20) & 0xFFu) : -1 - lane;
    const int c2 = dT2 ? (int)(sl.y & 0xFFFFu) : 0, c1 = dT1 ? (int)(sl.y >> 16) : 0;
    const uint32_t ordc = ((uint32_t)(BP_MAX_RANK - (int)(sl.z & 0xFFu)) << 16) | (uint32_t)(BP_MAX_RANK - (int)((sl.z >> 8) & 0xFFu));
    int bval[RC];
    uint32_t bord[RC], bmid[RC];
#pragma unroll
    for (int q = 0; q < RC; ++q) { bval[q] = NEG_INF; bord[q] = 0; bmid[q] = 0; }
    const int rowbytes = k0 * 4;
    constexpr int U = COOP == 2 ? PAIR_MAX_INDEG : (RC >= 4 ? 4 : 8);
    for (int t = t_lo; t < t_hi; t += U) {
        if (act) {
            int vals[U][RC], dl[U];
#pragma unroll
            for (int u = 0; u < U; ++u) {
                if (t + u < t_hi) {
                    const uint32_t px = (uint32_t)__builtin_amdgcn_readlane((int)rec.x, t + u), py = (uint32_t)__builtin_amdgcn_readlane((int)rec.y, t + u);
                    const int iu = (int)(px & 0x7FFFu), w = (int)((px >> 15) & 1u) + (int)((px >> 24) & 1u) + wv;
                    const int off = ((iu * RP + (r0 - w)) * k0 + j) * 4 + pad_bytes;
                    dl[u] = (int)dm2[(int)(py & 0x7FFu) * dT2 + c2] + (int)dm1[(int)((py >> 11) & 0x7FFu) * dT1 + c1];
#pragma unroll
                    for (int q = 0; q < RC; ++q) vals[u][q] = __builtin_amdgcn_raw_buffer_load_b32(cur_rsrc, off + q * rowbytes, 0, 0);
                }
            }
#pragma unroll
            for (int u = 0; u < U; ++u) {
                if (t + u < t_hi) {
                    const uint32_t px = (uint32_t)__builtin_amdgcn_readlane((int)rec.x, t + u), py = (uint32_t)__builtin_amdgcn_readlane((int)rec.y, t + u);
                    const int w = (int)((px >> 15) & 1u) + (int)((px >> 24) & 1u) + wv;
                    const uint32_t ord = ((uint32_t)(BP_MAX_RANK - (int)((py >> 22) & RANK_MASK)) << 24) | ((uint32_t)(BP_MAX_RANK - (int)((py >> RU1_SHIFT) & RANK_MASK)) << 8) | ordc;
                    const uint32_t mid = ((((px >> 16) & 0xFFu) << 16) | ((px >> 24) & 1u)) + lanemid;
                    relax_pair<RC>(vals[u], dl[u], ord, mid, r0, w, RP, bval, bord, bmid);
                }
            }
        }
    }
    if (COOP == 2) {
        if (part > 0) {
#pragma unroll
            for (int q = 0; q < RC; ++q) ex[((part - 1) * RC + q) * 64 + lane] = make_uint4((uint32_t)bval[q], bord[q], bmid[q], 0u);
        }
        __syncthreads();
        if (part > 0) return;
#pragma unroll
        for (int p = 0; p < 3; ++p) {
#pragma unroll
            for (int q = 0; q < RC; ++q) {
                const uint4 o = ex[(p * RC + q) * 64 + lane];
                merge_best_pair((int)o.x, o.y, o.z, true, bval[q], bord[q], bmid[q]);
            }
        }
    }
    if (steps > 0) {
        const int oj2 = lane_down1(j2);
        const bool same = (lane + 1 < 64) & (oj2 == j2);
#pragma unroll
        for (int q = 0; q < RC; ++q) merge_best_pair(lane_down1(bval[q]), (uint32_t)lane_down1((int)bord[q]), (uint32_t)lane_down1((int)bmid[q]), same, bval[q], bord[q], bmid[q]);
    }
    for (int st = 1, sh = 2; st < steps; ++st, sh <<= 1) {
        const int oj2 = __shfl_down(j2, sh);
        const bool same = (lane + sh < 64) & (oj2 == j2);
#pragma unroll
        for (int q = 0; q < RC; ++q)
            merge_best_pair(__shfl_down(bval[q], sh), (uint32_t)__shfl_down((int)bord[q], sh), (uint32_t)__shfl_down((int)bmid[q], sh), same, bval[q], bord[q], bmid[q]);
    }
    const int pj2 = lane_up1(j2);
    const bool head = act & ((lane == 0) | (pj2 != j2));
    unsigned long long dsum = 0;
    if (head) {
        const int k1 = kk & 0xFF, k2 = kk >> 8;
#pragma unroll
        for (int q = 0; q < RC; ++q) {
            const int r2 = r0 + q;
            if (r2 < RP) {
                const int idx = (i2 * RP + r2) * k2 + j2;
                nxt[idx] = bval[q];
                if (bp2) {
                    const uint32_t b2 = ~(bord[q] >> 16);
                    if (nt) store_bp_nt(&bp2[idx], b2); else bp2[idx] = (uint16_t)b2;
                    if (bord[q]) {
                        const uint32_t m = bmid[q];
                        bp1[((int)(m >> 16) * RP + r2 - (int)(m & 0xFFu)) * k1 + (int)((m >> 8) & 0xFFu)] = (uint16_t)~bord[q];
                    }
                }
                if (DIGEST && bval[q] != NEG_INF) {
                    const unsigned long long o = ((unsigned long long)r2 * k2 + i2) * k2 + j2;
                    dsum += digest_term(bval[q], o, bmid[q] >> 16, (bmid[q] >> 8) & 0xFFu);
                }
            }
        }
    }
    if (DIGEST && dsum) atomicAdd(&digest[lvl], dsum);
}

template <int RC, typename... DG>
__global__ __launch_bounds__(256) void dp_sweep_pair_kernel(const uint2 *prow_l, const uint4 *pslots_l, const int32_t *cur, const uint16_t *dm1, const uint16_t *dm2,
                                                            int nblocks, int rp_k, int pad_bytes, int dT1, int dT2, uint32_t buf_bytes,
                                                            int32_t *__restrict__ nxt, uint16_t *__restrict__ bp1, uint16_t *__restrict__ bp2, int kk, int nt, int *progress, int lvl,
                                                            DG... digest) {
    constexpr bool DIGEST = sizeof...(DG) != 0;
    publish_level(progress, lvl);
    const int g = (int)blockIdx.x * 4 + (int)(threadIdx.x >> 6), r0 = (int)blockIdx.y * RC, i2 = (int)blockIdx.z;
    if (g >= nblocks) return;
    const PairHead H{pslots_l, cur, dm1, dm2, rp_k & 0x1FFF, rp_k >> 13, pad_bytes, dT1, dT2, buf_bytes};
    unsigned long long *const acc[] = {nullptr, digest...};
    pair_task<RC, DIGEST, 0>(H, prow_l + i2 * PAIR_MAX_INDEG, nxt, bp1, bp2, kk, nt, i2, g, r0, lvl, acc[sizeof...(DG)]);
}

template <int RC, typename... DG>
__global__ __launch_bounds__(256) void dp_sweep_pair_coop_kernel(const uint2 *prow_l, const uint4 *pslots_l, const uint2 *pbig_l, const int32_t *cur, const uint16_t *dm2,
                                                                 unsigned long long big_in, int nblocks, int n_big, int rp_k, int dT2,
                                                                 const uint16_t *dm1, int dT1, int pad_bytes, uint32_t buf_bytes, const int32_t *__restrict__ big_rows,
                                                                 int32_t *__restrict__ nxt, uint16_t *__restrict__ bp1, uint16_t *__restrict__ bp2, int kk, int nt, int *progress, int lvl,
                                                                 DG... digest) {
    constexpr bool DIGEST = sizeof...(DG) != 0;
    publish_level(progress, lvl);
    const PairHead H{pslots_l, cur, dm1, dm2, rp_k & 0x1FFF, rp_k >> 13, pad_bytes, dT1, dT2, buf_bytes};
    unsigned long long *const acc[] = {nullptr, digest...};
    const int r0 = (int)blockIdx.y * RC;
    const int zc = 4 * n_big;
    if ((int)blockIdx.z < zc) {
        __shared__ uint4 ex[3 * RC * 64];
        const int hz = (int)blockIdx.z;
        const int g = (int)blockIdx.x * 4 + (hz & 3);
        if (g >= nblocks) return;
        const int h = hz >> 2;
        const int i2 = h < PAIR_BIG_INLINE ? (int)((big_in >> (8 * h)) & 0xFFu) : big_rows[h];
        pair_task<RC, DIGEST, 2>(H, pbig_l + h * PAIR_BIG_MAX_INDEG, nxt, bp1, bp2, kk, nt, i2, g, r0, lvl, acc[sizeof...(DG)], (int)(threadIdx.x >> 6), ex);
        return;
    }
    const int g = (int)blockIdx.x * 4 + (int)(threadIdx.x >> 6), i2 = (int)blockIdx.z - zc;
    if (g >= nblocks) return;
    pair_task<RC, DIGEST, 1>(H, prow_l + i2 * PAIR_MAX_INDEG, nxt, bp1, bp2, kk, nt, i2, g, r0, lvl, acc[sizeof...(DG)]);
}

constexpr int WARM_RANGES = 5;
struct WarmRanges { const char *p[WARM_RANGES]; long long n16[WARM_RANGES]; };
__global__ __launch_bounds__(256) void dp_warm_tables_kernel(WarmRanges W) {
    const long long tid = (long long)blockIdx.x * blockDim.x + threadIdx.x, nth = (long long)gridDim.x * blockDim.x;
#pragma unroll
    for (int q = 0; q < WARM_RANGES; ++q) {
        const uint4 *p = (const uint4 *)W.p[q];
        for (long long i = tid; i < W.n16[q]; i += nth) { uint4 v = p[i]; asm volatile("" ::"v"(v.x), "v"(v.y), "v"(v.z), "v"(v.w)); }
    }
}

constexpr int PF_WORKGROUPS = 16, PF_FAR_WORKGROUPS = 16;
constexpr unsigned long long PF_IDLE_TICKS = 30000;
struct PfCtl { int seq, stop, levels_done, probe, probe_ok, pad_[27]; int level; int pad2_[31]; };

__global__ void dp_pf_ctl_kernel(PfCtl *c, int seq, int level, int stop) {
    __hip_atomic_store(&c->level, level, __ATOMIC_RELAXED, __HIP_MEMORY_SCOPE_AGENT);
    __hip_atomic_store(&c->stop, stop, __ATOMIC_RELAXED, __HIP_MEMORY_SCOPE_AGENT);
    __hip_atomic_store(&c->seq, seq, __ATOMIC_RELEASE, __HIP_MEMORY_SCOPE_AGENT);
}

__global__ void dp_pf_probe_wait_kernel(PfCtl *c, int token) {
    const unsigned long long t0 = __builtin_amdgcn_s_memrealtime();
    int ok = 0;
    while (__builtin_amdgcn_s_memrealtime() - t0 < 200000ULL) {
        if (__hip_atomic_load(&c->probe, __ATOMIC_RELAXED, __HIP_MEMORY_SCOPE_AGENT) == token) { ok = 1; break; }
        __builtin_amdgcn_s_sleep(16);
    }
    c->probe_ok = ok;
}
__global__ void dp_pf_probe_set_kernel(PfCtl *c, int token) { __hip_atomic_store(&c->probe, token, __ATOMIC_RELAXED, __HIP_MEMORY_SCOPE_AGENT); }

__global__ __launch_bounds__(64) void dp_l2_prefetch_kernel(const LevelDesc *__restrict__ descs, FastArgs F, PfCtl *ctl, int seq, int lb, int le, int ahead_near, int delta_resident, int far,
                                                            const int32_t *__restrict__ pair_at, const PairDesc *__restrict__ pairs, const uint2 *__restrict__ prow, const uint4 *__restrict__ pslots, const uint2 *__restrict__ pbig) {
    __shared__ int dump[64];
#define DG_DROP_LOAD(PTR) __builtin_amdgcn_global_load_lds((const __attribute__((address_space(1))) void *)(PTR), (__attribute__((address_space(3))) void *)dump, 4, 0, 0)
    const bool far_role = (int)blockIdx.x >= PF_WORKGROUPS;
    const int lane = (int)threadIdx.x;
    const int slot = far_role ? (int)blockIdx.x - PF_WORKGROUPS : (int)(blockIdx.x >> 3), nslot = far_role ? (int)gridDim.x - PF_WORKGROUPS : PF_WORKGROUPS >> 3;
    const int ahead = far_role ? far : ahead_near, behind = far_role ? far - 64 : 0;
    int last = INT32_MIN, done = 0;
    unsigned long long t_last = __builtin_amdgcn_s_memrealtime();
    int *level_word = &ctl->level;
    auto lines = [&](const char *base, long long bytes) {
        if (bytes <= 0) return;
        const uintptr_t a = (uintptr_t)base & ~(uintptr_t)127;
        const int n = (int)(((uintptr_t)base + (uintptr_t)bytes - a + 127) >> 7);
        for (int t = slot * 64 + lane; t < n; t += nslot * 64) DG_DROP_LOAD((const char *)a + ((size_t)t << 7));
    };
    int polls = 0;
    for (int lp = lb; lp < le;) {
        if ((polls++ & 31) == 0 &&
            (__hip_atomic_load(&ctl->seq, __ATOMIC_ACQUIRE, __HIP_MEMORY_SCOPE_AGENT) != seq || __hip_atomic_load(&ctl->stop, __ATOMIC_RELAXED, __HIP_MEMORY_SCOPE_AGENT))) break;
        const int lv = __builtin_amdgcn_readfirstlane(__hip_atomic_load(level_word, __ATOMIC_RELAXED, __HIP_MEMORY_SCOPE_AGENT));
        const unsigned long long now = __builtin_amdgcn_s_memrealtime();
        if (lv != last) { last = lv; t_last = now; } else if (now - t_last > PF_IDLE_TICKS) break;
        if (lp <= lv + behind) lp = lv + behind + 1;
        if (lp >= le) break;
        if (lp - lv > ahead) { __builtin_amdgcn_s_sleep(48); continue; }
        const LevelDesc &d = descs[lp];
        const int k2 = __builtin_amdgcn_readfirstlane(d.k2), T = __builtin_amdgcn_readfirstlane(d.T);
        const int pa = pair_at ? __builtin_amdgcn_readfirstlane(pair_at[lp]) : -1;
        if (pa == -2) { ++lp; ++done; continue; }
        if (pa >= 0) {
            const PairDesc &p = pairs[pa];
            lines((const char *)(prow + p.row_first), 8LL * PAIR_MAX_INDEG * k2);
            lines((const char *)(pslots + p.slot_first), 1024LL * p.nblocks);
            lines((const char *)(pbig + (long long)PAIR_BIG_MAX_INDEG * p.big_first), 8LL * PAIR_BIG_MAX_INDEG * p.n_big);
            if (delta_resident) {
                const LevelDesc &d1 = descs[lp - 1];
                if (d.delta_off >= 0 && (long long)T * T <= (128 << 10)) lines((const char *)(F.delta + d.delta_off), 2LL * T * T);
                if (d1.delta_off >= 0 && (long long)d1.T * d1.T <= (128 << 10)) lines((const char *)(F.delta + d1.delta_off), 2LL * d1.T * d1.T);
            }
            ++lp; ++done;
            continue;
        }
        lines((const char *)(F.rowrec + d.b0), 16LL * k2);
        lines((const char *)(F.slots + d.slot_first), 512LL * d.nblocks);
        lines((const char *)(F.in_edge + d.in_base), 4LL * T);
        if (d.rowx_stride > 0) lines((const char *)(F.rowx + d.rowx_off), 4LL * k2 * d.rowx_stride);
        if (delta_resident && d.delta_off >= 0 && (long long)T * T <= (128 << 10)) lines((const char *)(F.delta + d.delta_off), 2LL * T * T);
        ++lp; ++done;
    }
    if (lane == 0 && blockIdx.x == 0) atomicAdd(&ctl->levels_done, done);
#undef DG_DROP_LOAD
}

enum : unsigned { RC_COOP = 1, RC_PART = 2, RC_ALL = 4, RC_ANY = 7 };
constexpr struct SweepRc { int rc; unsigned is; } SWEEP_RCS[] = {
    {1, RC_COOP | RC_PART}, {2, RC_COOP | RC_PART}, {3, RC_COOP | RC_PART}, {4, RC_COOP | RC_PART}, {5, RC_PART}, {6, RC_PART},
    {8, RC_PART | RC_ALL}, {10, RC_PART}, {11, RC_PART}, {16, RC_PART}, {19, RC_ALL}, {33, RC_ALL}};
constexpr int N_SWEEP_RCS = (int)(sizeof SWEEP_RCS / sizeof SWEEP_RCS[0]);
constexpr bool sweep_rcs_ascend(int q = 1) { return q >= N_SWEEP_RCS || (SWEEP_RCS[q - 1].rc < SWEEP_RCS[q].rc && sweep_rcs_ascend(q + 1)); }
static_assert(SWEEP_RCS[0].rc >= 1 && sweep_rcs_ascend() && (SWEEP_RCS[N_SWEEP_RCS - 1].is & RC_ALL), "ascending (choose_rc's ties go to the larger RC), and the largest chunk is an all-planes one");

int SweepVariant::count() { return 1 + 4 * N_SWEEP_RCS; }
SweepVariant SweepVariant::at(int index) { return index == 0 ? SweepVariant{0, false, false} : SweepVariant{SWEEP_RCS[(index - 1) / 4].rc, ((index - 1) & 2) != 0, ((index - 1) & 1) != 0}; }
int SweepVariant::index() const {
    for (int q = 0; q < N_SWEEP_RCS; ++q) if (SWEEP_RCS[q].rc == rc) return 1 + 4 * q + (general ? 2 : 0) + (coop ? 1 : 0);
    return 0;
}
bool SweepVariant::exists() const {
    if (rc == 0) return !general && !coop;
    for (const SweepRc &e : SWEEP_RCS) if (e.rc == rc) return !coop || (e.is & RC_COOP);
    return false;
}
std::string SweepVariant::name() const {
    return rc == 0 ? "dp_sweep_kernel" : std::string("dp_sweep_") + (coop ? "coop" : "fast") + "_kernel<" + std::to_string(rc) + (general ? ",general>" : ",lean>");
}

template <unsigned WANT, int Q = 0, class F>
static bool launch_variant(int rc, bool digest, bool general, F &f) {
    if constexpr (Q < N_SWEEP_RCS) {
        if constexpr ((SWEEP_RCS[Q].is & WANT) != 0) if (rc == SWEEP_RCS[Q].rc) {
            constexpr std::integral_constant<int, SWEEP_RCS[Q].rc> RC{};
            if (digest) { if (general) f(RC, std::true_type{}, std::true_type{}); else f(RC, std::true_type{}, std::false_type{}); }
            else { if (general) f(RC, std::false_type{}, std::true_type{}); else f(RC, std::false_type{}, std::false_type{}); }
            return true;
        }
        return launch_variant<WANT, Q + 1>(rc, digest, general, f);
    }
    return false;
}

void sweep_prepare(const DpState &S, SweepLaunch &X) {
    for (const SweepRc &e : SWEEP_RCS) if ((e.is & RC_ALL) && (X.rc_sel = e.rc) >= S.RP) break;
    X.digest = S.opt.want_digest != 0; X.rp_active = S.RP;
    X.small_state = S.state_alloc_bytes < ((size_t)1 << 31);
    SweepArgs &A = X.A;
    A.descs = S.d_descs.as<LevelDesc>(); A.in_off = S.d_in_off.as<uint32_t>(); A.in_edge = S.d_in_edge.as<uint32_t>();
    A.grp_begin = S.d_grp.as<uint32_t>(); A.in_dst = S.d_in_dst.as<int32_t>(); A.dead_cols = S.d_dead.as<int32_t>();
    A.delta = A.delta_zero = S.d_delta.as<uint16_t>();
    A.ring = S.d_ring.as<char>(); A.slot_bytes = S.state_alloc_bytes; A.pad_bytes = 4 * (size_t)S.pad_front;
    A.bp = nullptr; A.digest = S.d_digest.as<unsigned long long>(); A.RP = S.RP; A.flip = 0;
    FastArgs &F = X.F;
    F.rowrec = S.d_rowrec.as<uint4>(); F.slots = S.d_slots.as<uint2>(); F.in_edge = A.in_edge; F.rowx = S.d_rowx.as<uint32_t>(); F.dead_cols = A.dead_cols;
    F.delta = F.delta_zero = A.delta; F.bp = nullptr; F.digest = A.digest; F.RP = S.RP;
    F.ring = S.d_ring.as<char>(); F.slot_bytes = (uint32_t)S.state_alloc_bytes; F.flip = 0;
#ifdef DG_SWEEP_PROBE
    F.probe = S.d_probe.as<unsigned long long>();
#endif
    F.progress = A.progress = &S.d_pfctl.as<PfCtl>()->level;
    F.pad_bytes = (int)(4 * S.pad_front);
    F.buf_bytes = (uint32_t)std::min<size_t>(S.state_alloc_bytes, 0x7FFFFFFFu);
}

void sweep_init_state(const DpState &S, hipStream_t s) {
    hipLaunchKernelGGL(dp_init_kernel, dim3((unsigned)((S.RP + 255) / 256)), dim3(256), 0, s, S.d_ring.as<int32_t>() + S.pad_front, S.RP);
}

static void choose_rc(const DpState &S, const SweepLaunch &X, const LevelDesc &d, int l, int &rc, bool &coop) {
    const int rc_sel = rc = X.rc_sel;
    coop = false;
    if (S.opt.adaptive_rc == 0) return;
    const bool coop_ok = S.opt.use_coop && d.n_heavy > 0 && d.k2 + 4 * d.n_heavy <= 65535;
    const double dmax = (double)std::max(1, S.level_dmax[l]);
    double best = 1e300;
    for (int pass = (coop_ok && S.opt.use_coop == 2) ? 1 : 0; pass < (coop_ok ? 2 : 1); ++pass) {
        for (const SweepRc &e : SWEEP_RCS) {
            if (e.rc != rc_sel && !((e.is & RC_PART) && e.rc < rc_sel)) continue;
            if (pass == 1 && !(e.is & RC_COOP)) continue;
            if (S.opt.test_force_rc && e.rc != S.opt.test_force_rc) continue;
            const double rows = pass ? (double)d.k2 + 4.0 * d.n_heavy : (double)d.k2;
            const double chain = pass ? std::max((double)COOP_MIN, std::ceil(dmax / 4.0)) + 1.0 : dmax;
            const double W = rows * d.nblocks * ((X.rp_active + e.rc - 1) / e.rc);
            const double T = std::max(1.0, W / (double)S.opt.rc_cap) * ((double)S.opt.rc_t0_ns + chain * e.rc * (double)S.opt.rc_tg_ps * 1e-3) + W * (double)S.opt.rc_tw_ps * 1e-3;
            if (T <= best) { best = T; rc = e.rc; coop = pass == 1; }
        }
    }
}

int sweep_launch_level(const DpState &S, SweepLaunch &X, int l, hipStream_t s) {
    LevelDesc d = S.descs[l];
    d.bp_nt = (int64_t)d.k2 * d.k2 * S.RP >= S.opt.bp_nt_min_cells ? 1 : 0;
    SweepVariant v{0, false, false};
    bool launched;
    if (d.fast_ok && X.small_state && S.RP <= 65535 && S.opt.use_fast) {
        choose_rc(S, X, d, l, v.rc, v.coop);
        v.general = d.fast_ok == 2;
        const int nch = (X.rp_active + v.rc - 1) / v.rc;
        const dim3 grid((unsigned)((d.nblocks + 3) / 4), (unsigned)nch, (unsigned)(d.k2 + (v.coop ? 4 * d.n_heavy : 0)));
        const dim3 pgrid((unsigned)((d.nblocks + DG_PLAIN_GW - 1) / DG_PLAIN_GW), (unsigned)((nch + DG_PLAIN_CH - 1) / DG_PLAIN_CH), grid.z);
        const int32_t *hv = S.d_heavy.as<int32_t>();
        FastArgs F = X.F;
        F.flip = X.flip;
        const uint4 *rowrec_l = F.rowrec + d.b0;
        const uint2 *slots_l = F.slots + d.slot_first;
        const uint32_t *rowx_l = F.rowx + d.rowx_off;
        const int32_t *cur = (const int32_t *)(F.ring + (size_t)(DG_SLOT(l - 1) ^ X.flip) * F.slot_bytes);
        const int dT = d.delta_off >= 0 ? d.T : 0;
        const uint16_t *dm = dT ? F.delta + d.delta_off - (int64_t)d.in_base * dT : F.delta_zero;
        const int rp_k = S.RP | (d.k << 13);
        unsigned long long hlo = 0, hhi = 0;
        for (int q = 0; q < 4; ++q) { hlo |= (unsigned long long)(uint16_t)d.heavy_in[q] << (16 * q); hhi |= (unsigned long long)(uint16_t)d.heavy_in[4 + q] << (16 * q); }
        auto fast = [&](auto RC, auto DG, auto GEN) { hipLaunchKernelGGL((dp_sweep_fast_kernel<RC.value, DG.value, GEN.value>), pgrid, dim3(DG_PLAIN_WG), 0, s, rowrec_l, slots_l, rowx_l, cur, dm, d.rowx_stride, d.nblocks, rp_k, F.pad_bytes, dT, F.buf_bytes, F, d, l); };
        auto cooperative = [&](auto RC, auto DG, auto GEN) { hipLaunchKernelGGL((dp_sweep_coop_kernel<RC.value, DG.value, GEN.value>), grid, dim3(256), 0, s, rowrec_l, slots_l, rowx_l, cur, d.rowx_stride, d.nblocks, d.n_heavy, rp_k, hlo, hhi, F, d, l, dm, dT, hv); };
        launched = v.coop ? launch_variant<RC_COOP>(v.rc, X.digest, v.general, cooperative) : launch_variant<RC_ANY>(v.rc, X.digest, v.general, fast);
    } else {
        const int nchunk = (S.RP + X.rc_sel - 1) / X.rc_sel;
        const int64_t ntask = (int64_t)d.k2 * d.ngroups * nchunk;
        const unsigned grid = (unsigned)std::min<int64_t>((ntask + 3) / 4, S.opt.max_blocks);
        SweepArgs A = X.A;
        A.flip = X.flip;
        auto generic = [&](auto RC, auto DG, auto) { hipLaunchKernelGGL((dp_sweep_kernel<RC.value, DG.value>), dim3(grid), dim3(256), 0, s, A, l); };
        launched = launch_variant<RC_ALL>(X.rc_sel, X.digest, false, generic);
    }
    if (!launched) { set_error("sweep of level %d: no %s kernel is instantiated for chunks of %d recombination counts", l, v.coop ? "cooperative" : v.rc ? "fast" : "generic", v.rc ? v.rc : X.rc_sel); return DG_ERR_STATE; }
    X.hist.n[(size_t)v.index()]++;
    return DG_OK;
}

static int choose_pair_rc(const DpState &S, const PairDesc &p) {
    for (int q = 0; q < N_PAIR_RCS; ++q) if (S.opt.test_force_pair_rc == PAIR_RCS[q]) return q;
    int best_q = 0;
    double best = 1e300;
    const double rows = (double)p.k2 + 4.0 * p.n_big;
    const double chain = p.n_big ? std::max((double)p.dmax_light, std::ceil(p.dmax / 4.0) + 1.0) : (double)p.dmax;
    for (int q = 0; q < N_PAIR_RCS; ++q) {
        const int rc = PAIR_RCS[q];
        const double W = rows * p.nblocks * ((S.RP + rc - 1) / rc);
        const double T = std::max(1.0, W / (double)S.opt.rc_cap) * ((double)S.opt.rc_t0_ns + chain * rc * (double)S.opt.rc_tg_ps * 1e-3) + W * (double)S.opt.rc_tw_ps * 1e-3;
        if (T <= best) { best = T; best_q = q; }
    }
    return best_q;
}
std::string pair_variant_name(int q) { return std::string(q < N_PAIR_RCS ? "dp_sweep_pair_kernel<" : "dp_sweep_pair_coop_kernel<") + std::to_string(PAIR_RCS[q % N_PAIR_RCS]) + ">"; }

template <int Q = 0, class F>
static void launch_pair_rc(int q, bool digest, F &f) {
    if constexpr (Q < N_PAIR_RCS) {
        if (q != Q) return launch_pair_rc<Q + 1>(q, digest, f);
        constexpr std::integral_constant<int, PAIR_RCS[Q]> RC{};
        if (digest) f(RC, std::true_type{}); else f(RC, std::false_type{});
    }
}

int sweep_launch_pair(const DpState &S, SweepLaunch &X, int l, hipStream_t s) {
    const PairDesc &p = S.pairs[(size_t)S.pair_at[l]];
    const LevelDesc &d2 = S.descs[l], &d1 = S.descs[l - 1];
    const FastArgs &F = X.F;
    const int q = choose_pair_rc(S, p), rc = PAIR_RCS[q];
    const int nch = (S.RP + rc - 1) / rc;
    const dim3 grid((unsigned)((p.nblocks + 3) / 4), (unsigned)nch, (unsigned)(p.k2 + 4 * p.n_big));
    const int32_t *cur = (const int32_t *)(F.ring + (size_t)(DG_SLOT(l - 2) ^ X.flip) * F.slot_bytes);
    int32_t *nxt = (int32_t *)(F.ring + (size_t)(DG_SLOT(l - 1) ^ X.flip) * F.slot_bytes + F.pad_bytes);
    const int dT1 = d1.delta_off >= 0 ? d1.T : 0, dT2 = d2.delta_off >= 0 ? d2.T : 0;
    const uint16_t *dm1 = dT1 ? F.delta + d1.delta_off : F.delta_zero, *dm2 = dT2 ? F.delta + d2.delta_off : F.delta_zero;
    const int nt = (int64_t)d2.k2 * d2.k2 * S.RP >= S.opt.bp_nt_min_cells ? 1 : 0;
    const uint2 *prow_l = S.d_prow.as<uint2>() + p.row_first;
    const uint4 *pslots_l = S.d_pslots.as<uint4>() + p.slot_first;
    const int rp_k = S.RP | (p.k0 << 13), kk = p.k1 | (p.k2 << 8), nblocks = p.nblocks, n_big = p.n_big, pad_bytes = F.pad_bytes;
    const uint32_t buf_bytes = F.buf_bytes;
    uint16_t *bp1 = F.bp ? F.bp + d1.bp_off : nullptr, *bp2 = F.bp ? F.bp + d2.bp_off : nullptr;
    int *progress = F.progress;
    unsigned long long *digest = F.digest;
    if (p.n_big == 0) {
        auto light = [&](auto RC, auto DG) {
            if constexpr (DG.value) hipLaunchKernelGGL((dp_sweep_pair_kernel<RC.value, unsigned long long *>), grid, dim3(256), 0, s, prow_l, pslots_l, cur, dm1, dm2, nblocks, rp_k, pad_bytes, dT1, dT2, buf_bytes, nxt, bp1, bp2, kk, nt, progress, l, digest);
            else hipLaunchKernelGGL((dp_sweep_pair_kernel<RC.value>), grid, dim3(256), 0, s, prow_l, pslots_l, cur, dm1, dm2, nblocks, rp_k, pad_bytes, dT1, dT2, buf_bytes, nxt, bp1, bp2, kk, nt, progress, l);
        };
        launch_pair_rc(q, X.digest, light);
    } else {
        const uint2 *pbig_l = S.d_pbig.as<uint2>() + (size_t)PAIR_BIG_MAX_INDEG * (size_t)p.big_first;
        const int32_t *big_rows = S.d_pbig_rows.as<int32_t>() + p.big_first;
        unsigned long long big_in = 0;
        for (int h = 0; h < PAIR_BIG_INLINE; ++h) big_in |= (unsigned long long)p.big_in[h] << (8 * h);
        auto fanin = [&](auto RC, auto DG) {
            if constexpr (DG.value) hipLaunchKernelGGL((dp_sweep_pair_coop_kernel<RC.value, unsigned long long *>), grid, dim3(256), 0, s, prow_l, pslots_l, pbig_l, cur, dm2, big_in, nblocks, n_big, rp_k, dT2, dm1, dT1, pad_bytes, buf_bytes, big_rows, nxt, bp1, bp2, kk, nt, progress, l, digest);
            else hipLaunchKernelGGL((dp_sweep_pair_coop_kernel<RC.value>), grid, dim3(256), 0, s, prow_l, pslots_l, pbig_l, cur, dm2, big_in, nblocks, n_big, rp_k, dT2, dm1, dT1, pad_bytes, buf_bytes, big_rows, nxt, bp1, bp2, kk, nt, progress, l);
        };
        launch_pair_rc(q, X.digest, fanin);
    }
    X.flip ^= 1;
    X.pair_hist.n[q + (p.n_big ? N_PAIR_RCS : 0)]++;
    return DG_OK;
}

void sweep_warm_tables(const DpState &S, const SweepLaunch &X, int q0, int q1, hipStream_t s) {
    const LevelDesc &da = S.descs[q0], &db = S.descs[q1 - 1];
    const FastArgs &F = X.F;
    WarmRanges W{};
    auto put = [&](int q, const void *base, int64_t b0, int64_t b1) {
        const uintptr_t a = ((uintptr_t)base + (uintptr_t)b0) & ~(uintptr_t)15, e = ((uintptr_t)base + (uintptr_t)b1) & ~(uintptr_t)15;
        W.p[q] = (const char *)a; W.n16[q] = e > a ? (long long)((e - a) >> 4) : 0;
    };
    put(0, F.rowrec, 16 * (int64_t)da.b0, 16 * ((int64_t)db.b0 + db.k2));
    put(1, F.slots, 8 * da.slot_first, 8 * (db.slot_first + (int64_t)db.nblocks * 64));
    put(2, F.in_edge, 4 * (int64_t)da.in_base, 4 * ((int64_t)db.in_base + db.T));
    int64_t d0 = -1, d1 = -1, x0 = -1, x1 = -1;
    for (int q = q0; q < q1; ++q) {
        const LevelDesc &dq = S.descs[q];
        if (dq.rowx_stride > 0) {
            if (x0 < 0) x0 = dq.rowx_off;
            x1 = dq.rowx_off + (int64_t)dq.k2 * dq.rowx_stride;
        }
        if (dq.delta_off < 0 || S.level_win[q] != S.cur_win) continue;
        const int64_t e = dq.delta_off + (int64_t)dq.T * dq.T;
        d0 = d0 < 0 ? dq.delta_off : std::min(d0, dq.delta_off);
        d1 = std::max(d1, e);
    }
    if (d0 >= 0) put(3, F.delta, 2 * d0, 2 * d1);
    if (x0 >= 0) put(4, F.rowx, 4 * x0, 4 * x1);
    long long tot = 0;
    for (int q = 0; q < WARM_RANGES; ++q) tot += W.n16[q];
    if (tot <= 0) return;
    const unsigned grid = (unsigned)std::min<long long>((tot + 255) / 256, 2048);
    hipLaunchKernelGGL(dp_warm_tables_kernel, dim3(grid), dim3(256), 0, s, W);
}

int sweep_prefetch_begin(DpState &S, const SweepLaunch &X, int lb, int le, bool delta_resident, hipStream_t s) {
    S.pf_active = false;
    if (S.opt.l2_prefetch <= 0 || !X.small_state || !S.opt.use_fast || le - lb < 64) return DG_OK;
    if (!S.pf_stream && hipStreamCreateWithFlags(&S.pf_stream, hipStreamNonBlocking) != hipSuccess) { (void)hipGetLastError(); S.pf_stream = nullptr; S.opt.l2_prefetch = 0; return DG_OK; }
    if (!S.pf_ev && hipEventCreateWithFlags(&S.pf_ev, hipEventDisableTiming) != hipSuccess) { (void)hipGetLastError(); S.pf_ev = nullptr; S.opt.l2_prefetch = 0; return DG_OK; }
    if (!S.side_stream_ok()) return DG_OK;
    if (!S.pf_tested) {
        S.pf_tested = 1;
        DG_HIP(hipStreamSynchronize(s));
        hipLaunchKernelGGL(dp_pf_probe_wait_kernel, dim3(1), dim3(1), 0, S.pf_stream, S.d_pfctl.as<PfCtl>(), 0x5EED);
        hipLaunchKernelGGL(dp_pf_probe_set_kernel, dim3(1), dim3(1), 0, s, S.d_pfctl.as<PfCtl>(), 0x5EED);
        PfCtl h;
        if (hipStreamSynchronize(S.pf_stream) != hipSuccess || hipStreamSynchronize(s) != hipSuccess ||
            hipMemcpy(&h, S.d_pfctl.p, sizeof h, hipMemcpyDeviceToHost) != hipSuccess || !h.probe_ok) {
            (void)hipGetLastError();
            if (getenv("DG_DEBUG")) fprintf(stderr, "[dipgenie_hip] L2 prefetcher off: its stream does not run beside the sweep's\n");
            S.opt.l2_prefetch = 0;
            return DG_OK;
        }
    }
    const int seq = ++S.pf_seq;
    hipLaunchKernelGGL(dp_pf_ctl_kernel, dim3(1), dim3(1), 0, s, S.d_pfctl.as<PfCtl>(), seq, lb - 1, 0);
    DG_HIP(hipEventRecord(S.pf_ev, s));
    DG_HIP(hipStreamWaitEvent(S.pf_stream, S.pf_ev, 0));
    const int far = (int)S.opt.pf_far;
    hipLaunchKernelGGL(dp_l2_prefetch_kernel, dim3(PF_WORKGROUPS + (far > 0 ? PF_FAR_WORKGROUPS : 0)), dim3(64), 0, S.pf_stream, S.d_descs.as<LevelDesc>(), X.F,
                       S.d_pfctl.as<PfCtl>(), seq, lb, le, (int)S.opt.l2_prefetch, delta_resident ? 1 : 0, far,
                       X.pairs_ok ? S.d_pair_at.as<int32_t>() : (const int32_t *)nullptr, S.d_pairs.as<PairDesc>(), S.d_prow.as<uint2>(), S.d_pslots.as<uint4>(), S.d_pbig.as<uint2>());
    S.pf_active = true;
    return DG_OK;
}
void sweep_prefetch_end(DpState &S, int le, hipStream_t s) {
    if (S.pf_stream && S.opt.l2_prefetch > 0) hipLaunchKernelGGL(dp_pf_ctl_kernel, dim3(1), dim3(1), 0, s, S.d_pfctl.as<PfCtl>(), S.pf_seq, le, 1);
}
void sweep_prefetch_free(DpState &S) {
    if (S.pf_stream) { (void)hipStreamSynchronize(S.pf_stream); (void)hipStreamDestroy(S.pf_stream); S.pf_stream = nullptr; }
    if (S.pf_ev) { (void)hipEventDestroy(S.pf_ev); S.pf_ev = nullptr; }
}

}
```

Before: 67.66 billion.

## Add wide bit-packing layout so level pairing covers levels up to width 1023

Introduces a second record bit layout (templated on WIDE) for the fused two-level pair sweep, so levels whose width exceeds 255 (up to 1023) can also be paired instead of falling back to per-level launches. The pair chooser now tries a wide-enabled selection and adopts it when enough wide pairs are found, and the kernels and launch paths are instantiated for both layouts. This cuts kernel launches and intermediate state traffic for wide graphs, at the cost of narrower bit fields (mid-row width limited to 3 bits, fewer inline big rows) and extra kernel instantiations.

```diff
diff --git a/dipgenie_amd/csrc/dg_dp.hpp b/dipgenie_amd/csrc/dg_dp.hpp
--- a/dipgenie_amd/csrc/dg_dp.hpp
+++ b/dipgenie_amd/csrc/dg_dp.hpp
@@ -103,6 +103,11 @@
 constexpr int PAIR_BIG_MAX_INDEG = 32;
 constexpr int PAIR_BIG_INLINE = 8;
 constexpr uint32_t PAIR_ROW_BIG = 15;
+constexpr int PAIR_WIDE_MAX_WIDTH = 1023;
+constexpr int PAIR_WIDE_BIG_INLINE = 4;
+template <bool WIDE> struct PairLayout;
+template <> struct PairLayout<false> { static constexpr uint32_t POS = 0x7FFFu, W1 = 15, MID = 16, MID_MASK = 0xFFu, W2 = 24, DEG = 25, COL_MASK = 0xFFu, MID_ROW = 16, MID_COL = 8, MID_W = 0xFFu, KK = 8; };
+template <> struct PairLayout<true> { static constexpr uint32_t POS = 0x3FFu, W1 = 10, MID = 11, MID_MASK = 0x3FFu, W2 = 21, DEG = 22, COL_MASK = 0x3FFu, MID_ROW = 13, MID_COL = 3, MID_W = 0x7u, KK = 10; };
 struct PairDesc {
     int32_t l, nblocks;
     int32_t k0, k1, k2;
@@ -111,11 +116,13 @@
     int64_t slot_first;
     int32_t n_big, dmax_light;
     int64_t big_first;
-    uint8_t big_in[PAIR_BIG_INLINE];
-};
+    uint16_t big_in[PAIR_BIG_INLINE];
+    int32_t wide;
+};
+constexpr int PAIR_HIST_WIDE = 2 * N_PAIR_RCS, N_PAIR_HIST = 2 * PAIR_HIST_WIDE;
 struct PairHist {
-    int64_t n[2 * N_PAIR_RCS] = {};
-    void add(const PairHist &o, int64_t sign = 1) { for (int q = 0; q < 2 * N_PAIR_RCS; ++q) n[q] += sign * o.n[q]; }
+    int64_t n[N_PAIR_HIST] = {};
+    void add(const PairHist &o, int64_t sign = 1) { for (int q = 0; q < N_PAIR_HIST; ++q) n[q] += sign * o.n[q]; }
 };
 
 struct SweepHist {
@@ -156,6 +163,11 @@
     int64_t pair_fanin = 1;
     int64_t pair_fanin_min = 4096;
     int64_t pair_fanin_max_big = 4, pair_fanin_max_indeg = PAIR_BIG_MAX_INDEG;
+    int64_t pair_wide = 1;
+    int64_t pair_wide_min = 1024;
+    int64_t pair_wide_fanin = 1;
+    int64_t pair_wide_max_width = PAIR_WIDE_MAX_WIDTH;
+    int64_t pair_wide_rc = 0;
     int64_t pair_digest = 0;
     int64_t test_force_pair_rc = 0;
     int64_t joint_state_bytes = (int64_t)8 << 30;
diff --git a/dipgenie_amd/csrc/dg_dp_pairs.hip b/dipgenie_amd/csrc/dg_dp_pairs.hip
--- a/dipgenie_amd/csrc/dg_dp_pairs.hip
+++ b/dipgenie_amd/csrc/dg_dp_pairs.hip
@@ -48,9 +48,10 @@
     DG_HIP(hipStreamSynchronize(c->stream));
     const int nt = (int)std::max<int64_t>(1, std::min<int64_t>({(int64_t)16, S.opt.host_threads, (int64_t)cpu_share()}));
     auto indeg = [&](int v) { return (int)(in_off[v + 1] - in_off[v]); };
+    const int wide_cap = (int)std::min<int64_t>(S.opt.pair_wide_max_width, PAIR_WIDE_MAX_WIDTH), any_cap = S.opt.pair_wide ? std::max(wide_cap, PAIR_MAX_WIDTH) : PAIR_MAX_WIDTH;
     auto level_ok = [&](int l) {
         const LevelDesc &d = S.descs[l];
-        return d.fast_ok == 1 && d.ndead == 0 && d.k2 <= PAIR_MAX_WIDTH && d.T <= PAIR_MAX_T && !d.bp_wide;
+        return d.fast_ok == 1 && d.ndead == 0 && d.k2 <= any_cap && d.T <= PAIR_MAX_T && !d.bp_wide;
     };
     struct LevelSum { int32_t cmin, cmax, cmax_light, n_big; };
     std::vector<uint16_t> comp((size_t)nV, 0);
@@ -71,17 +72,21 @@
         }
     });
     const int max_big = (int)std::min<int64_t>(S.opt.pair_fanin_max_big, PAIR_MAX_WIDTH), max_indeg = (int)std::min<int64_t>(S.opt.pair_fanin_max_indeg, PAIR_BIG_MAX_INDEG);
-    auto choose = [&](bool fanin, std::vector<PairDesc> &pairs, std::vector<int32_t> &at) {
+    auto choose = [&](bool fanin, bool wide, std::vector<PairDesc> &pairs, std::vector<int32_t> &at, int64_t &n_wide) {
         int64_t n_fanin = 0;
+        n_wide = 0;
         pairs.clear(); at.assign((size_t)L, -1);
         for (int l = 2; l < L; ++l) {
             const LevelSum &s = sum[(size_t)l];
             if (s.cmin < 1) continue;
-            if (s.cmax > PAIR_MAX_INDEG && !(fanin && s.cmax <= max_indeg && s.n_big <= max_big)) continue;
             const LevelDesc &d = S.descs[l];
+            const int k0 = S.descs[l - 1].k;
+            const bool wide_level = d.k > PAIR_MAX_WIDTH || d.k2 > PAIR_MAX_WIDTH, wide_layout = wide_level || (wide && k0 > PAIR_MAX_WIDTH && k0 <= wide_cap);
+            if (wide_level && !(wide && k0 <= wide_cap && d.k <= wide_cap && d.k2 <= wide_cap)) continue;
+            if (s.cmax > PAIR_MAX_INDEG && !(fanin && s.cmax <= max_indeg && s.n_big <= max_big && !(wide_layout && !S.opt.pair_wide_fanin))) continue;
             PairDesc p{};
-            p.l = l; p.k0 = S.descs[l - 1].k; p.k1 = d.k; p.k2 = d.k2; p.dmax = s.cmax; p.n_big = s.n_big; p.dmax_light = s.cmax_light;
-            n_fanin += s.n_big > 0;
+            p.l = l; p.k0 = k0; p.k1 = d.k; p.k2 = d.k2; p.dmax = s.cmax; p.n_big = s.n_big; p.dmax_light = s.cmax_light; p.wide = wide_layout;
+            n_fanin += s.n_big > 0; n_wide += wide_layout;
             at[(size_t)l] = (int32_t)pairs.size(); at[(size_t)l - 1] = -2;
             pairs.push_back(p);
             ++l;
@@ -90,12 +95,23 @@
     };
     std::vector<int32_t> at;
     std::vector<PairDesc> pairs;
-    int64_t n_fanin = choose(false, pairs, at);
-    if (S.opt.pair_fanin) {
+    int64_t n_fanin = 0, n_wide = 0;
+    auto choose_fanin = [&](bool wide, std::vector<PairDesc> &pairs, std::vector<int32_t> &at, int64_t &n_fanin, int64_t &n_wide) {
+        n_fanin = choose(false, wide, pairs, at, n_wide);
+        if (!S.opt.pair_fanin) return;
         std::vector<int32_t> at_f;
         std::vector<PairDesc> pairs_f;
-        const int64_t nf = choose(true, pairs_f, at_f);
-        if (nf >= std::max<int64_t>(S.opt.pair_fanin_min, 1)) { pairs.swap(pairs_f); at.swap(at_f); n_fanin = nf; }
+        int64_t nw = 0;
+        const int64_t nf = choose(true, wide, pairs_f, at_f, nw);
+        if (nf >= std::max<int64_t>(S.opt.pair_fanin_min, 1)) { pairs.swap(pairs_f); at.swap(at_f); n_fanin = nf; n_wide = nw; }
+    };
+    choose_fanin(false, pairs, at, n_fanin, n_wide);
+    if (S.opt.pair_wide) {
+        std::vector<int32_t> at_w;
+        std::vector<PairDesc> pairs_w;
+        int64_t nf = 0, nw = 0;
+        choose_fanin(true, pairs_w, at_w, nf, nw);
+        if (nw >= std::max<int64_t>(S.opt.pair_wide_min, 1)) { pairs.swap(pairs_w); at.swap(at_w); n_fanin = nf; n_wide = nw; }
     }
     if ((int64_t)pairs.size() < std::max<int64_t>(S.opt.pair_min, 1)) return DG_OK;
     const int64_t NP = (int64_t)pairs.size();
@@ -129,6 +145,9 @@
             uint32_t *blk = pslots.get() + 4 * p.slot_first;
             int32_t *const br = big_rows.get() + p.big_first;
             uint32_t used = 0, maxdv = 1, h = 0;
+            typedef PairLayout<false> Y0;
+            typedef PairLayout<true> Y1;
+            const uint32_t W1 = p.wide ? Y1::W1 : Y0::W1, MID = p.wide ? Y1::MID : Y0::MID, W2 = p.wide ? Y1::W2 : Y0::W2, DEG = p.wide ? Y1::DEG : Y0::DEG;
             auto close_block = [&]() {
                 uint32_t steps = 0;
                 while ((1u << steps) < maxdv) ++steps;
@@ -151,20 +170,20 @@
                     for (uint32_t e1 = in_off[mv]; e1 < in_off[mv + 1]; ++e1, ++t) {
                         const uint32_t src = in_edge[e1] & 0x7FFFu, w1 = in_edge[e1] >> 31, r1 = e1 - in_off[mv];
                         const uint32_t i2 = e2 - d2.in_base, i1 = e1 - d1.in_base;
-                        rec[2 * t] = src | (w1 << 15) | (m << 16) | (w2 << 24) | (n << 25);
+                        rec[2 * t] = src | (w1 << W1) | (m << MID) | (w2 << W2) | (n << DEG);
                         rec[2 * t + 1] = i2 | (i1 << 11) | (r2 << 22) | (r1 << ru1_shift);
                         uint32_t *const sl = blk + 4 * (used + t);
-                        sl[0] = src | (w1 << 15) | (m << 16) | (w2 << 24);
+                        sl[0] = src | (w1 << W1) | (m << MID) | (w2 << W2);
                         sl[1] = i2 | (i1 << 16);
                         sl[2] = r2 | (r1 << 8) | ((uint32_t)c2 << 20);
                         sl[3] = 0;
                     }
                 }
-                for (; t < cap; ++t) { rec[2 * t] = n << 25; rec[2 * t + 1] = 0; }
+                for (; t < cap; ++t) { rec[2 * t] = n << DEG; rec[2 * t + 1] = 0; }
                 if (big) {
-                    for (t = 0; t < (uint32_t)PAIR_MAX_INDEG; ++t) { light[2 * t] = PAIR_ROW_BIG << 25; light[2 * t + 1] = 0; }
+                    for (t = 0; t < (uint32_t)PAIR_MAX_INDEG; ++t) { light[2 * t] = PAIR_ROW_BIG << DEG; light[2 * t + 1] = 0; }
                     br[h] = c2;
-                    if (h < (uint32_t)PAIR_BIG_INLINE) p.big_in[h] = (uint8_t)c2;
+                    if (h < (uint32_t)PAIR_BIG_INLINE) p.big_in[h] = (uint16_t)c2;
                     ++h;
                 }
                 used += n; maxdv = std::max(maxdv, n);
@@ -185,8 +204,8 @@
     if (int rc = up(S.d_pbig_rows, big_rows.get(), 4 * (size_t)n_big)) return rc;
     DG_HIP(hipStreamSynchronize(c->stream));
     if (getenv("DG_DEBUG"))
-        fprintf(stderr, "[dipgenie_hip] load: %zu level pairs (%.1f %% of the launches), %lld of them with big rows (%lld big rows), composed tables %.1f MB, built in %.3f s by %d threads\n",
-                pairs.size(), 100.0 * (double)pairs.size() / std::max(1, L - 1), (long long)n_fanin, (long long)n_big, 4e-6 * (double)(prow_words + pslot_words + pbig_words), wall_s() - t0, nt);
+        fprintf(stderr, "[dipgenie_hip] load: %zu level pairs (%.1f %% of the launches), %lld of them with big rows (%lld big rows), %lld in the wide layout, composed tables %.1f MB, built in %.3f s by %d threads\n",
+                pairs.size(), 100.0 * (double)pairs.size() / std::max(1, L - 1), (long long)n_fanin, (long long)n_big, (long long)n_wide, 4e-6 * (double)(prow_words + pslot_words + pbig_words), wall_s() - t0, nt);
     S.pairs.swap(pairs); S.pair_at.swap(at);
     return DG_OK;
 }
diff --git a/dipgenie_amd/csrc/dg_dp_run.hip b/dipgenie_amd/csrc/dg_dp_run.hip
--- a/dipgenie_amd/csrc/dg_dp_run.hip
+++ b/dipgenie_amd/csrc/dg_dp_run.hip
@@ -491,7 +491,7 @@
 extern "C" int dg_dp_get_pair_profile(dg_ctx *c, char *buf, int cap) {
     if (!c || !c->dp || !buf || cap < 2) { dgi::set_error("dg_dp_get_pair_profile: no state"); return DG_ERR_STATE; }
     std::string out;
-    for (int q = 0; q < 2 * dgi::N_PAIR_RCS; ++q)
+    for (int q = 0; q < dgi::N_PAIR_HIST; ++q)
         if (const int64_t n = c->dp->pair_hist.n[q]) out += (out.empty() ? "" : " ") + dgi::pair_variant_name(q) + ':' + std::to_string(n);
     if ((int)out.size() + 1 > cap) { dgi::set_error("dg_dp_get_pair_profile: buffer too small (%zu needed)", out.size() + 1); return DG_ERR_ARG; }
     memcpy(buf, out.c_str(), out.size() + 1);
@@ -520,6 +520,7 @@
     {"graph_batch", &DpO::graph_batch, -1, false}, {"l2_prefetch", &DpO::l2_prefetch, 0, false}, {"delta_overlap", &DpO::delta_overlap, 0, false}, {"pf_far", &DpO::pf_far, 0, false},
     {"side_stream", &DpO::side_stream, -1, false}, {"plane_limit", &DpO::plane_limit, 0, false}, {"test_poison_level", &DpO::test_poison_level, 0, false},
     {"test_poison_byte", &DpO::test_poison_byte, 0, false}, {"test_force_rc", &DpO::test_force_rc, 0, false}, {"pair_digest", &DpO::pair_digest, 0, false}, {"test_force_pair_rc", &DpO::test_force_pair_rc, 0, false},
+    {"pair_wide_rc", &DpO::pair_wide_rc, 0, false},
     {"score_slab_bytes", &DpO::score_slab_bytes, 0, true}, {"partner_slab_bytes", &DpO::partner_slab_bytes, 0, true},
     {"partner_wide", &DpO::partner_wide, 0, false},
     {"joint_state_bytes", &DpO::joint_state_bytes, 0, true},
@@ -530,6 +531,8 @@
     {"host_threads", &DpO::host_threads, 1, false}, {"host_tables", &DpO::host_tables, 0, false}, {"delta_cap_entries", &DpO::delta_cap_entries, 0, true},
     {"pair_levels", &DpO::pair_levels, 0, false}, {"pair_min", &DpO::pair_min, 1, false}, {"pair_fanin", &DpO::pair_fanin, 0, false}, {"pair_fanin_min", &DpO::pair_fanin_min, 1, false},
     {"pair_fanin_max_big", &DpO::pair_fanin_max_big, 0, false}, {"pair_fanin_max_indeg", &DpO::pair_fanin_max_indeg, 0, false},
+    {"pair_wide", &DpO::pair_wide, 0, false}, {"pair_wide_min", &DpO::pair_wide_min, 1, false}, {"pair_wide_fanin", &DpO::pair_wide_fanin, 0, false},
+    {"pair_wide_max_width", &DpO::pair_wide_max_width, 0, true},
     {"lattice_chunk_cells", &DpO::chunk_units_cfg, 1, false},
 };
 static int dp_option(dg_ctx *c, const char *what, const char *key, const int64_t *set, int64_t *get) {
diff --git a/dipgenie_amd/csrc/dg_dp_sweep.hip b/dipgenie_amd/csrc/dg_dp_sweep.hip
--- a/dipgenie_amd/csrc/dg_dp_sweep.hip
+++ b/dipgenie_amd/csrc/dg_dp_sweep.hip
@@ -449,9 +449,10 @@
     uint32_t buf_bytes;
 };
 
-template <int RC, bool DIGEST, int COOP>
+template <int RC, bool DIGEST, int COOP, bool WIDE>
 __device__ __forceinline__ void pair_task(const PairHead &H, const uint2 *recs, int32_t *__restrict__ nxt, uint16_t *__restrict__ bp1, uint16_t *__restrict__ bp2, int kk, int nt,
                                           int i2, int g, int r0, int lvl, unsigned long long *digest, int part = 0, uint4 *ex = nullptr) {
+    typedef PairLayout<WIDE> Y;
     const int lane = threadIdx.x & 63;
     const int RP = H.RP, k0 = H.k0, pad_bytes = H.pad_bytes, dT1 = H.dT1, dT2 = H.dT2;
     const uint16_t *dm1 = H.dm1, *dm2 = H.dm2;
@@ -459,14 +460,14 @@
     const uint2 rec = recs[lane & (NREC - 1)];
     const uint4 sl = H.pslots_l[g * 64 + lane];
     const __amdgpu_buffer_rsrc_t cur_rsrc = state_rsrc(H.cur, H.buf_bytes);
-    const int du = __builtin_amdgcn_readfirstlane((int)(rec.x >> 25)) & (COOP == 2 ? 0x3F : 0xF);
+    const int du = __builtin_amdgcn_readfirstlane((int)(rec.x >> Y::DEG)) & (COOP == 2 ? 0x3F : 0xF);
     if (COOP == 1 && du > PAIR_MAX_INDEG) return;
     const int t_lo = COOP == 2 ? (du * part) >> 2 : 0, t_hi = COOP == 2 ? (du * (part + 1)) >> 2 : du;
     const int steps = __builtin_amdgcn_readfirstlane((int)(sl.z >> 16)) & 0xF;
     const bool act = sl.x != 0xFFFFFFFFu;
-    const int j = (int)(sl.x & 0x7FFFu), wv = (int)((sl.x >> 15) & 1u) + (int)((sl.x >> 24) & 1u);
-    const uint32_t lanemid = (((sl.x >> 16) & 0xFFu) << 8) | ((sl.x >> 24) & 1u);
-    const int j2 = act ? (int)((sl.z >> 20) & 0xFFu) : -1 - lane;
+    const int j = (int)(sl.x & Y::POS), wv = (int)((sl.x >> Y::W1) & 1u) + (int)((sl.x >> Y::W2) & 1u);
+    const uint32_t lanemid = (((sl.x >> Y::MID) & Y::MID_MASK) << Y::MID_COL) | ((sl.x >> Y::W2) & 1u);
+    const int j2 = act ? (int)((sl.z >> 20) & Y::COL_MASK) : -1 - lane;
     const int c2 = dT2 ? (int)(sl.y & 0xFFFFu) : 0, c1 = dT1 ? (int)(sl.y >> 16) : 0;
     const uint32_t ordc = ((uint32_t)(BP_MAX_RANK - (int)(sl.z & 0xFFu)) << 16) | (uint32_t)(BP_MAX_RANK - (int)((sl.z >> 8) & 0xFFu));
     int bval[RC];
@@ -482,7 +483,7 @@
             for (int u = 0; u < U; ++u) {
                 if (t + u < t_hi) {
                     const uint32_t px = (uint32_t)__builtin_amdgcn_readlane((int)rec.x, t + u), py = (uint32_t)__builtin_amdgcn_readlane((int)rec.y, t + u);
-                    const int iu = (int)(px & 0x7FFFu), w = (int)((px >> 15) & 1u) + (int)((px >> 24) & 1u) + wv;
+                    const int iu = (int)(px & Y::POS), w = (int)((px >> Y::W1) & 1u) + (int)((px >> Y::W2) & 1u) + wv;
                     const int off = ((iu * RP + (r0 - w)) * k0 + j) * 4 + pad_bytes;
                     dl[u] = (int)dm2[(int)(py & 0x7FFu) * dT2 + c2] + (int)dm1[(int)((py >> 11) & 0x7FFu) * dT1 + c1];
 #pragma unroll
@@ -493,9 +494,9 @@
             for (int u = 0; u < U; ++u) {
                 if (t + u < t_hi) {
                     const uint32_t px = (uint32_t)__builtin_amdgcn_readlane((int)rec.x, t + u), py = (uint32_t)__builtin_amdgcn_readlane((int)rec.y, t + u);
-                    const int w = (int)((px >> 15) & 1u) + (int)((px >> 24) & 1u) + wv;
+                    const int w = (int)((px >> Y::W1) & 1u) + (int)((px >> Y::W2) & 1u) + wv;
                     const uint32_t ord = ((uint32_t)(BP_MAX_RANK - (int)((py >> 22) & RANK_MASK)) << 24) | ((uint32_t)(BP_MAX_RANK - (int)((py >> RU1_SHIFT) & RANK_MASK)) << 8) | ordc;
-                    const uint32_t mid = ((((px >> 16) & 0xFFu) << 16) | ((px >> 24) & 1u)) + lanemid;
+                    const uint32_t mid = ((((px >> Y::MID) & Y::MID_MASK) << Y::MID_ROW) | ((px >> Y::W2) & 1u)) + lanemid;
                     relax_pair<RC>(vals[u], dl[u], ord, mid, r0, w, RP, bval, bord, bmid);
                 }
             }
@@ -534,7 +535,7 @@
     const bool head = act & ((lane == 0) | (pj2 != j2));
     unsigned long long dsum = 0;
     if (head) {
-        const int k1 = kk & 0xFF, k2 = kk >> 8;
+        const int k1 = kk & (int)Y::COL_MASK, k2 = kk >> Y::KK;
 #pragma unroll
         for (int q = 0; q < RC; ++q) {
             const int r2 = r0 + q;
@@ -546,12 +547,12 @@
                     if (nt) store_bp_nt(&bp2[idx], b2); else bp2[idx] = (uint16_t)b2;
                     if (bord[q]) {
                         const uint32_t m = bmid[q];
-                        bp1[((int)(m >> 16) * RP + r2 - (int)(m & 0xFFu)) * k1 + (int)((m >> 8) & 0xFFu)] = (uint16_t)~bord[q];
+                        bp1[((int)(m >> Y::MID_ROW) * RP + r2 - (int)(m & Y::MID_W)) * k1 + (int)((m >> Y::MID_COL) & Y::MID_MASK)] = (uint16_t)~bord[q];
                     }
                 }
                 if (DIGEST && bval[q] != NEG_INF) {
                     const unsigned long long o = ((unsigned long long)r2 * k2 + i2) * k2 + j2;
-                    dsum += digest_term(bval[q], o, bmid[q] >> 16, (bmid[q] >> 8) & 0xFFu);
+                    dsum += digest_term(bval[q], o, bmid[q] >> Y::MID_ROW, (bmid[q] >> Y::MID_COL) & Y::MID_MASK);
                 }
             }
         }
@@ -559,7 +560,7 @@
     if (DIGEST && dsum) atomicAdd(&digest[lvl], dsum);
 }
 
-template <int RC, typename... DG>
+template <int RC, bool WIDE, typename... DG>
 __global__ __launch_bounds__(256) void dp_sweep_pair_kernel(const uint2 *prow_l, const uint4 *pslots_l, const int32_t *cur, const uint16_t *dm1, const uint16_t *dm2,
                                                             int nblocks, int rp_k, int pad_bytes, int dT1, int dT2, uint32_t buf_bytes,
                                                             int32_t *__restrict__ nxt, uint16_t *__restrict__ bp1, uint16_t *__restrict__ bp2, int kk, int nt, int *progress, int lvl,
@@ -570,10 +571,10 @@
     if (g >= nblocks) return;
     const PairHead H{pslots_l, cur, dm1, dm2, rp_k & 0x1FFF, rp_k >> 13, pad_bytes, dT1, dT2, buf_bytes};
     unsigned long long *const acc[] = {nullptr, digest...};
-    pair_task<RC, DIGEST, 0>(H, prow_l + i2 * PAIR_MAX_INDEG, nxt, bp1, bp2, kk, nt, i2, g, r0, lvl, acc[sizeof...(DG)]);
-}
-
-template <int RC, typename... DG>
+    pair_task<RC, DIGEST, 0, WIDE>(H, prow_l + i2 * PAIR_MAX_INDEG, nxt, bp1, bp2, kk, nt, i2, g, r0, lvl, acc[sizeof...(DG)]);
+}
+
+template <int RC, bool WIDE, typename... DG>
 __global__ __launch_bounds__(256) void dp_sweep_pair_coop_kernel(const uint2 *prow_l, const uint4 *pslots_l, const uint2 *pbig_l, const int32_t *cur, const uint16_t *dm2,
                                                                  unsigned long long big_in, int nblocks, int n_big, int rp_k, int dT2,
                                                                  const uint16_t *dm1, int dT1, int pad_bytes, uint32_t buf_bytes, const int32_t *__restrict__ big_rows,
@@ -591,13 +592,14 @@
         const int g = (int)blockIdx.x * 4 + (hz & 3);
         if (g >= nblocks) return;
         const int h = hz >> 2;
-        const int i2 = h < PAIR_BIG_INLINE ? (int)((big_in >> (8 * h)) & 0xFFu) : big_rows[h];
-        pair_task<RC, DIGEST, 2>(H, pbig_l + h * PAIR_BIG_MAX_INDEG, nxt, bp1, bp2, kk, nt, i2, g, r0, lvl, acc[sizeof...(DG)], (int)(threadIdx.x >> 6), ex);
+        const int i2 = WIDE ? (h < PAIR_WIDE_BIG_INLINE ? (int)((big_in >> (16 * h)) & 0xFFFFu) : big_rows[h])
+                            : (h < PAIR_BIG_INLINE ? (int)((big_in >> (8 * h)) & 0xFFu) : big_rows[h]);
+        pair_task<RC, DIGEST, 2, WIDE>(H, pbig_l + h * PAIR_BIG_MAX_INDEG, nxt, bp1, bp2, kk, nt, i2, g, r0, lvl, acc[sizeof...(DG)], (int)(threadIdx.x >> 6), ex);
         return;
     }
     const int g = (int)blockIdx.x * 4 + (int)(threadIdx.x >> 6), i2 = (int)blockIdx.z - zc;
     if (g >= nblocks) return;
-    pair_task<RC, DIGEST, 1>(H, prow_l + i2 * PAIR_MAX_INDEG, nxt, bp1, bp2, kk, nt, i2, g, r0, lvl, acc[sizeof...(DG)]);
+    pair_task<RC, DIGEST, 1, WIDE>(H, prow_l + i2 * PAIR_MAX_INDEG, nxt, bp1, bp2, kk, nt, i2, g, r0, lvl, acc[sizeof...(DG)]);
 }
 
 constexpr int WARM_RANGES = 5;
@@ -813,6 +815,7 @@
 
 static int choose_pair_rc(const DpState &S, const PairDesc &p) {
     for (int q = 0; q < N_PAIR_RCS; ++q) if (S.opt.test_force_pair_rc == PAIR_RCS[q]) return q;
+    for (int q = 0; q < N_PAIR_RCS; ++q) if (p.wide && S.opt.pair_wide_rc == PAIR_RCS[q]) return q;
     int best_q = 0;
     double best = 1e300;
     const double rows = (double)p.k2 + 4.0 * p.n_big;
@@ -825,7 +828,10 @@
     }
     return best_q;
 }
-std::string pair_variant_name(int q) { return std::string(q < N_PAIR_RCS ? "dp_sweep_pair_kernel<" : "dp_sweep_pair_coop_kernel<") + std::to_string(PAIR_RCS[q % N_PAIR_RCS]) + ">"; }
+std::string pair_variant_name(int q) {
+    static const char *const kernels[] = {"dp_sweep_pair_kernel<", "dp_sweep_pair_coop_kernel<", "dp_sweep_pair_wide_kernel<", "dp_sweep_pair_coop_wide_kernel<"};
+    return std::string(kernels[q / N_PAIR_RCS]) + std::to_string(PAIR_RCS[q % N_PAIR_RCS]) + ">";
+}
 
 template <int Q = 0, class F>
 static void launch_pair_rc(int q, bool digest, F &f) {
@@ -850,30 +856,39 @@
     const int nt = (int64_t)d2.k2 * d2.k2 * S.RP >= S.opt.bp_nt_min_cells ? 1 : 0;
     const uint2 *prow_l = S.d_prow.as<uint2>() + p.row_first;
     const uint4 *pslots_l = S.d_pslots.as<uint4>() + p.slot_first;
-    const int rp_k = S.RP | (p.k0 << 13), kk = p.k1 | (p.k2 << 8), nblocks = p.nblocks, n_big = p.n_big, pad_bytes = F.pad_bytes;
+    const int rp_k = S.RP | (p.k0 << 13), kk = p.k1 | (p.k2 << (p.wide ? PairLayout<true>::KK : PairLayout<false>::KK)), nblocks = p.nblocks, n_big = p.n_big, pad_bytes = F.pad_bytes;
     const uint32_t buf_bytes = F.buf_bytes;
     uint16_t *bp1 = F.bp ? F.bp + d1.bp_off : nullptr, *bp2 = F.bp ? F.bp + d2.bp_off : nullptr;
     int *progress = F.progress;
     unsigned long long *digest = F.digest;
     if (p.n_big == 0) {
         auto light = [&](auto RC, auto DG) {
-            if constexpr (DG.value) hipLaunchKernelGGL((dp_sweep_pair_kernel<RC.value, unsigned long long *>), grid, dim3(256), 0, s, prow_l, pslots_l, cur, dm1, dm2, nblocks, rp_k, pad_bytes, dT1, dT2, buf_bytes, nxt, bp1, bp2, kk, nt, progress, l, digest);
-            else hipLaunchKernelGGL((dp_sweep_pair_kernel<RC.value>), grid, dim3(256), 0, s, prow_l, pslots_l, cur, dm1, dm2, nblocks, rp_k, pad_bytes, dT1, dT2, buf_bytes, nxt, bp1, bp2, kk, nt, progress, l);
+            if constexpr (DG.value) hipLaunchKernelGGL((dp_sweep_pair_kernel<RC.value, false, unsigned long long *>), grid, dim3(256), 0, s, prow_l, pslots_l, cur, dm1, dm2, nblocks, rp_k, pad_bytes, dT1, dT2, buf_bytes, nxt, bp1, bp2, kk, nt, progress, l, digest);
+            else hipLaunchKernelGGL((dp_sweep_pair_kernel<RC.value, false>), grid, dim3(256), 0, s, prow_l, pslots_l, cur, dm1, dm2, nblocks, rp_k, pad_bytes, dT1, dT2, buf_bytes, nxt, bp1, bp2, kk, nt, progress, l);
         };
-        launch_pair_rc(q, X.digest, light);
+        auto light_wide = [&](auto RC, auto DG) {
+            if constexpr (DG.value) hipLaunchKernelGGL((dp_sweep_pair_kernel<RC.value, true, unsigned long long *>), grid, dim3(256), 0, s, prow_l, pslots_l, cur, dm1, dm2, nblocks, rp_k, pad_bytes, dT1, dT2, buf_bytes, nxt, bp1, bp2, kk, nt, progress, l, digest);
+            else hipLaunchKernelGGL((dp_sweep_pair_kernel<RC.value, true>), grid, dim3(256), 0, s, prow_l, pslots_l, cur, dm1, dm2, nblocks, rp_k, pad_bytes, dT1, dT2, buf_bytes, nxt, bp1, bp2, kk, nt, progress, l);
+        };
+        if (p.wide) launch_pair_rc(q, X.digest, light_wide); else launch_pair_rc(q, X.digest, light);
     } else {
         const uint2 *pbig_l = S.d_pbig.as<uint2>() + (size_t)PAIR_BIG_MAX_INDEG * (size_t)p.big_first;
         const int32_t *big_rows = S.d_pbig_rows.as<int32_t>() + p.big_first;
         unsigned long long big_in = 0;
-        for (int h = 0; h < PAIR_BIG_INLINE; ++h) big_in |= (unsigned long long)p.big_in[h] << (8 * h);
+        if (p.wide) for (int h = 0; h < PAIR_WIDE_BIG_INLINE; ++h) big_in |= (unsigned long long)p.big_in[h] << (16 * h);
+        else for (int h = 0; h < PAIR_BIG_INLINE; ++h) big_in |= (unsigned long long)p.big_in[h] << (8 * h);
         auto fanin = [&](auto RC, auto DG) {
-            if constexpr (DG.value) hipLaunchKernelGGL((dp_sweep_pair_coop_kernel<RC.value, unsigned long long *>), grid, dim3(256), 0, s, prow_l, pslots_l, pbig_l, cur, dm2, big_in, nblocks, n_big, rp_k, dT2, dm1, dT1, pad_bytes, buf_bytes, big_rows, nxt, bp1, bp2, kk, nt, progress, l, digest);
-            else hipLaunchKernelGGL((dp_sweep_pair_coop_kernel<RC.value>), grid, dim3(256), 0, s, prow_l, pslots_l, pbig_l, cur, dm2, big_in, nblocks, n_big, rp_k, dT2, dm1, dT1, pad_bytes, buf_bytes, big_rows, nxt, bp1, bp2, kk, nt, progress, l);
+            if constexpr (DG.value) hipLaunchKernelGGL((dp_sweep_pair_coop_kernel<RC.value, false, unsigned long long *>), grid, dim3(256), 0, s, prow_l, pslots_l, pbig_l, cur, dm2, big_in, nblocks, n_big, rp_k, dT2, dm1, dT1, pad_bytes, buf_bytes, big_rows, nxt, bp1, bp2, kk, nt, progress, l, digest);
+            else hipLaunchKernelGGL((dp_sweep_pair_coop_kernel<RC.value, false>), grid, dim3(256), 0, s, prow_l, pslots_l, pbig_l, cur, dm2, big_in, nblocks, n_big, rp_k, dT2, dm1, dT1, pad_bytes, buf_bytes, big_rows, nxt, bp1, bp2, kk, nt, progress, l);
         };
-        launch_pair_rc(q, X.digest, fanin);
+        auto fanin_wide = [&](auto RC, auto DG) {
+            if constexpr (DG.value) hipLaunchKernelGGL((dp_sweep_pair_coop_kernel<RC.value, true, unsigned long long *>), grid, dim3(256), 0, s, prow_l, pslots_l, pbig_l, cur, dm2, big_in, nblocks, n_big, rp_k, dT2, dm1, dT1, pad_bytes, buf_bytes, big_rows, nxt, bp1, bp2, kk, nt, progress, l, digest);
+            else hipLaunchKernelGGL((dp_sweep_pair_coop_kernel<RC.value, true>), grid, dim3(256), 0, s, prow_l, pslots_l, pbig_l, cur, dm2, big_in, nblocks, n_big, rp_k, dT2, dm1, dT1, pad_bytes, buf_bytes, big_rows, nxt, bp1, bp2, kk, nt, progress, l);
+        };
+        if (p.wide) launch_pair_rc(q, X.digest, fanin_wide); else launch_pair_rc(q, X.digest, fanin);
     }
     X.flip ^= 1;
-    X.pair_hist.n[q + (p.n_big ? N_PAIR_RCS : 0)]++;
+    X.pair_hist.n[q + (p.n_big ? N_PAIR_RCS : 0) + (p.wide ? PAIR_HIST_WIDE : 0)]++;
     return DG_OK;
 }
 
```

New measurement: 69.11 billion (median of 6 runs). 1.02x the previous value.
